# genomematt/xenomapper

Measured on AMD Instinct MI355X. Metric: read-pairs/sec classified, higher is better.
Workload: dtype int32; 1 GPU; configs[1]: 50000000 PE 2x150 pairs/GPU, AS/XS, liberal, HBM-resident; pairs_per_gpu=50000000, step=xm_classify_compact_dev: classify+count, scan, scatter (3 launches)

## Files before the change

### xenomapper_amd/build.py

```python
from __future__ import annotations

import os
import shutil
import subprocess
import sys

PKG = os.path.dirname(os.path.abspath(__file__))
REPO = os.path.dirname(PKG)
CSRC = os.path.join(PKG, "csrc")
HIP_LIB = os.path.join(PKG, "libxenomapper_hip.so")
HOST_LIB = os.path.join(PKG, "libxenomapper_host.so")

HIP_SOURCES = ["xm_kernels.hip", "xm_api.hip", "xm_strip.hip", "xm_inflate.hip", "xm_bamdev.hip"]
HOST_SOURCES = ["xm_sam.cpp", "xm_bam.cpp"]


def _hipcc():
    exe = shutil.which("hipcc") or "/opt/rocm/bin/hipcc"
    if not os.path.exists(exe):
        raise RuntimeError("hipcc not found: the HIP extension cannot be built")
    return exe


def _stale(target, sources):
    if not os.path.exists(target):
        return True
    t = os.path.getmtime(target)
    return any(os.path.getmtime(s) > t for s in sources)


def build_hip(force=False, verbose=False):
    srcs = [os.path.join(CSRC, s) for s in HIP_SOURCES]
    deps = srcs + [os.path.join(CSRC, "xm_kernels.h"), os.path.join(CSRC, "xm_inflate_core.h"),
                   os.path.join(CSRC, "xm_bamrec.h"), os.path.join(CSRC, "xm_fmtg.h"), os.path.join(CSRC, "xm_pinned.h"), os.path.join(CSRC, "xm_gather.h"),
                   os.path.join(REPO, "include", "xenomapper_hip.h"), os.path.join(REPO, "include", "xenomapper_strip.h"),
                   os.path.join(REPO, "include", "xenomapper_bgzf.h")]
    if not force and not _stale(HIP_LIB, deps):
        return HIP_LIB
    flags = ["-O3", "--offload-arch=gfx950", "-std=c++17", "-fPIC", "-Wall", "-Wextra", "-I", os.path.join(REPO, "include")] + \
        os.environ.get("XENOMAPPER_HIPCC_FLAGS", "").split()
    obj_dir = os.path.join(REPO, "build", "obj")
    os.makedirs(obj_dir, exist_ok=True)
    tag = os.path.join(obj_dir, "flags.txt")
    same_flags = os.path.exists(tag) and open(tag).read() == " ".join(flags)
    headers = deps[len(srcs):]
    jobs, objs = [], []
    for src in srcs:
        obj = os.path.join(obj_dir, os.path.basename(src) + ".o")
        objs.append(obj)
        if force or not same_flags or _stale(obj, [src] + headers):
            cmd = [_hipcc()] + flags + ["-c", src, "-o", obj]
            if verbose:
                print(" ".join(cmd), file=sys.stderr)
            jobs.append((cmd, subprocess.Popen(cmd)))
    failed = [cmd for cmd, proc in jobs if proc.wait() != 0]
    if failed:
        raise subprocess.CalledProcessError(1, failed[0])
    with open(tag, "w") as fh:
        fh.write(" ".join(flags))
    cmd = [_hipcc(), "--offload-arch=gfx950", "-shared", "-fPIC"] + objs + ["-o", HIP_LIB]
    if verbose:
        print(" ".join(cmd), file=sys.stderr)
    subprocess.check_call(cmd)
    return HIP_LIB


def build_host(force=False, verbose=False):
    srcs = [os.path.join(CSRC, s) for s in HOST_SOURCES]
    if not all(os.path.exists(s) for s in srcs):
        return None
    deps = srcs + [os.path.join(REPO, "include", "xenomapper_host.h"), os.path.join(CSRC, "xm_pool.h")]
    if not force and not _stale(HOST_LIB, deps):
        return HOST_LIB
    cmd = ["g++", "-O3", "-std=c++17", "-fPIC", "-shared", "-pthread", "-Wall", "-Wextra",
           "-I", os.path.join(REPO, "include")] + srcs + ["-o", HOST_LIB, "-lz", "-ldl"]
    if verbose:
        print(" ".join(cmd), file=sys.stderr)
    subprocess.check_call(cmd)
    return HOST_LIB


def build_host_sanitized(out_path, verbose=False):
    srcs = [os.path.join(CSRC, s) for s in HOST_SOURCES]
    cmd = ["g++", "-O1", "-g", "-std=c++17", "-fPIC", "-shared", "-pthread", "-fsanitize=address,undefined",
           "-fno-omit-frame-pointer", "-I", os.path.join(REPO, "include")] + srcs + ["-o", out_path, "-lz", "-ldl"]
    if verbose:
        print(" ".join(cmd), file=sys.stderr)
    subprocess.check_call(cmd)
    return out_path


def build_all(force=False, verbose=False):
    out = [build_hip(force, verbose)]
    host = build_host(force, verbose)
    if host:
        out.append(host)
    return out


if __name__ == "__main__":
    print("\n".join(build_all(force="--force" in sys.argv, verbose=True)))
```

### xenomapper_amd/csrc/xm_kernels.h

```cpp
#pragma once
#include <hip/hip_runtime.h>
#include <stdint.h>

#include "../../include/xenomapper_hip.h"

#define XM_BLOCK 256
#define XM_GRAN 2048
#define XM_MAX_GRANULES ((uint32_t)((0xFFFFF000ull + XM_GRAN - 1) / XM_GRAN))
#define XM_PART_GRAN 1024u
#define XM_PART_STRIDE 2112u
#define XM_PART_REPLICAS 64u
#define XM_COUNT_REPLICAS 64u
#define XM_CLASSIFY_BLOCK 512
#ifndef XM_CIGAR_BLOCK
#define XM_CIGAR_BLOCK 256
#endif
#define XM_CIGP_BLOCK 512
#ifndef XM_SCATTER_WAVES
#define XM_SCATTER_WAVES 1048576u
#endif
#define XM_CLASSIFY_NT true

namespace xm {

struct GranPlan {
    uint32_t n_gran;
    uint32_t gran_stride;
};

struct CountPlan {
    GranPlan plan = {0, 0};
    uint32_t *gran_counts = nullptr;
    uint32_t *part_tot = nullptr;
    uint8_t *bins4 = nullptr;
    uint64_t *counts_rep = nullptr;
    uint32_t gran0 = 0, gran1 = 0;
};

GranPlan plan_granules(uint64_t n);

struct CigCols {
    const int32_t *nm;
    const int32_t *xs;
    const uint8_t *cnt;
    const uint32_t *tile;
    const uint32_t *ops;
};

struct ListOut {
    uint32_t *p[7];
    uint32_t cap;
};

struct RunsOut {
    uint16_t *runs16;
    uint16_t *gran_counts16;
    uint64_t *counts_rep;
};
void launch_classify_runs_i32(hipStream_t st, int mode, uint64_t n,
                              const int32_t *as1, const int32_t *xs1, const int32_t *as2, const int32_t *xs2,
                              const uint64_t *unit_bits, int32_t m, const RunsOut &ro);
void launch_classify_runs_f64(hipStream_t st, int mode, uint64_t n,
                              const double *as1, const double *xs1, const double *as2, const double *xs2,
                              const uint64_t *unit_bits, double m, const RunsOut &ro);
void launch_runs_finish(hipStream_t st, int mode, uint64_t *counts_rep, uint64_t *counts, uint64_t *n_out);

void launch_classify_i32(hipStream_t st, int mode, uint64_t n,
                         const int32_t *as1, const int32_t *xs1, const int32_t *as2, const int32_t *xs2,
                         const uint64_t *unit_bits, int32_t m, uint8_t *code, const CountPlan *cp);
void launch_classify_f64(hipStream_t st, int mode, uint64_t n,
                         const double *as1, const double *xs1, const double *as2, const double *xs2,
                         const uint64_t *unit_bits, double m, uint8_t *code, const CountPlan *cp);
void launch_classify_cigar(hipStream_t st, int mode, uint64_t n,
                           const int32_t *nm1, const uint32_t *off1, const uint32_t *ops1, const int32_t *xs1,
                           const int32_t *nm2, const uint32_t *off2, const uint32_t *ops2, const int32_t *xs2,
                           const uint64_t *unit_bits, int32_t m, uint8_t *code, uint32_t *range_flag);
void launch_classify_cigp(hipStream_t st, int mode, uint64_t n, const CigCols &s1, const CigCols &s2,
                          const uint64_t *unit_bits, int32_t m, uint8_t *code, uint32_t *range_flag, const CountPlan &cp);
void launch_hist(hipStream_t st, int mode, uint64_t n, const uint8_t *code, const CountPlan &cp);
void launch_scan(hipStream_t st, const CountPlan &cp, uint32_t *gran_off, uint64_t *bin_totals, uint64_t *counts);
void launch_scatter(hipStream_t st, const GranPlan &p, int mode, uint64_t n, const uint8_t *code, bool code_is_bins4,
                    const uint32_t *gran_counts, const uint32_t *gran_off, const uint64_t *bin_totals, uint64_t *bin_offsets,
                    uint32_t *idx_out, uint32_t *part_tot, const ListOut *lists = nullptr, uint32_t gran0 = 0, uint32_t gran1 = 0);
void launch_stream_probe(hipStream_t st, uint64_t n, const int32_t *c0, const int32_t *c1, const int32_t *c2, const int32_t *c3,
                         uint8_t *out);
void launch_mate_correlate(hipStream_t st, uint64_t n, const double *track, uint32_t m, const double *density, double *out);
void launch_cigar(hipStream_t st, uint32_t max_blocks, uint64_t n, const int32_t *nm, const uint32_t *cig_off,
                  const uint32_t *cig_oplen, int32_t *as_out, uint32_t *range_flag);

}
```

### xenomapper_amd/csrc/xm_kernels.hip

```cpp
#include <hip/hip_runtime.h>
#include <stdint.h>
#include <stdlib.h>

#include "xm_kernels.h"

namespace xm {

template <typename T>
__device__ __forceinline__ uint32_t mapping_state(T a1, T x1, T a2, T x2, T m)
{
    const bool low1 = a1 <= m;
    const bool low2 = a2 <= m;
    const bool prim = (a1 > m) && (low2 || a1 > a2);
    const bool sec  = (a2 > m) && (low1 || a2 > a1);
    const bool spec1 = (x1 == T(0)) || (a1 > x1);
    const bool spec2 = (x2 == T(0)) || (a2 > x2);
    uint32_t s = 6u;
    s = sec ? (spec2 ? 1u : 3u) : s;
    s = (a1 == a2) ? 4u : s;
    s = prim ? (spec1 ? 0u : 2u) : s;
    s = (low1 && low2) ? 5u : s;
    return s;
}

template <>
__device__ __forceinline__ uint32_t mapping_state<int32_t>(int32_t a1, int32_t x1, int32_t a2, int32_t x2, int32_t m)
{
    const bool low1 = a1 <= m, low2 = a2 <= m;
    const bool gt = a1 > a2, lt = a2 > a1;
    const bool spec1 = (x1 == 0) || (a1 > x1);
    const bool spec2 = (x2 == 0) || (a2 > x2);
    uint32_t s = spec2 ? 1u : 3u;
    s = (gt || lt) ? s : 4u;
    s = (!low1 && (low2 || gt)) ? (spec1 ? 0u : 2u) : s;
    s = (low1 && low2) ? 5u : s;
    return s;
}

__device__ __forceinline__ uint32_t bin_of_code(int mode, uint32_t c)
{
    const uint32_t f = (c >> 3) & 7u, r = c & 7u;
    const uint32_t lo = f < r ? f : r;
    const uint32_t hi = f < r ? r : f;
    uint32_t b;
    if (mode == XM_MODE_SE) {
        b = r > 6u ? 6u : r;
    } else if (mode == XM_MODE_PE_LIBERAL) {
        b = lo;
    } else {
        b = (hi == 5u) ? 5u
          : ((hi == 4u) || (((f ^ r) & 1u) != 0u)) ? 4u
          : lo;
    }
    if (mode != XM_MODE_SE) b = (hi > 5u) ? 6u : b;
    return (c == XM_NO_UNIT) ? 7u : b;
}

template <typename T> struct Vec4;
typedef int32_t v4i32 __attribute__((ext_vector_type(4)));
typedef int32_t v4i32_a4 __attribute__((ext_vector_type(4), aligned(4)));
typedef double  v4f64 __attribute__((ext_vector_type(4)));
template <> struct Vec4<int32_t> { typedef v4i32 type; };
template <> struct Vec4<double>  { typedef v4f64 type; };

template <typename T> __device__ __forceinline__ T absent_value();
template <> __device__ __forceinline__ int32_t absent_value<int32_t>() { return INT32_MIN; }
template <> __device__ __forceinline__ double  absent_value<double>()  { return -__builtin_huge_val(); }

template <typename T, bool NT, bool FULL = false>
__device__ __forceinline__ void load4(const T *__restrict__ col, uint64_t r0, uint64_t n, T out[4])
{
    typedef typename Vec4<T>::type V;
    if (FULL || r0 + 4 <= n) {
        const V *p = reinterpret_cast<const V *>(col + r0);
        const V v = NT ? __builtin_nontemporal_load(p) : *p;
        out[0] = v.x; out[1] = v.y; out[2] = v.z; out[3] = v.w;
    } else {
#pragma unroll
        for (int j = 0; j < 4; ++j) out[j] = (r0 + j < n) ? col[r0 + j] : absent_value<T>();
    }
}

template <typename T, bool NT>
__device__ __forceinline__ void load4_wg(const T *__restrict__ wg, uint32_t byte_off, T out[4])
{
    typedef typename Vec4<T>::type V;
    const V *p = reinterpret_cast<const V *>(reinterpret_cast<const char *>(wg) + byte_off);
    const V v = NT ? __builtin_nontemporal_load(p) : *p;
    out[0] = v.x; out[1] = v.y; out[2] = v.z; out[3] = v.w;
}

__device__ __forceinline__ uint32_t wave_scan_incl(uint32_t v)
{
    v += (uint32_t)__builtin_amdgcn_update_dpp(0, (int)v, 0x111, 0xf, 0xf, false);
    v += (uint32_t)__builtin_amdgcn_update_dpp(0, (int)v, 0x112, 0xf, 0xf, false);
    v += (uint32_t)__builtin_amdgcn_update_dpp(0, (int)v, 0x114, 0xf, 0xf, false);
    v += (uint32_t)__builtin_amdgcn_update_dpp(0, (int)v, 0x118, 0xf, 0xf, false);
    v += (uint32_t)__builtin_amdgcn_update_dpp(0, (int)v, 0x142, 0xa, 0xf, false);
    v += (uint32_t)__builtin_amdgcn_update_dpp(0, (int)v, 0x143, 0xc, 0xf, false);
    return v;
}

__device__ __forceinline__ uint32_t lane_value(uint32_t v, int lane)
{
    return (uint32_t)__builtin_amdgcn_readlane((int)v, lane);
}

__device__ __forceinline__ void lds_settle()
{
    asm volatile("s_waitcnt lgkmcnt(0)" ::: "memory");
}

#define XM_HREP 8
#define XM_COUNT_LDS_WORDS (64 * XM_HREP + 16)

struct CountSink {
    uint32_t *gran_counts;
    uint32_t *part_tot;
    unsigned long long *counts_rep;
    uint8_t *bins4;
    uint32_t gran_stride;
    int mode;
    uint32_t blk0;
};

__device__ __forceinline__ void count_flush(uint32_t *lds, uint32_t granule, const CountSink &sink)
{
    const uint32_t lane = threadIdx.x & 63u;
    uint32_t *misc = lds + 64 * XM_HREP;
    const uint4 h0 = *reinterpret_cast<const uint4 *>(lds + lane * XM_HREP);
    const uint4 h1 = *reinterpret_cast<const uint4 *>(lds + lane * XM_HREP + 4);
    const uint32_t s = h0.x + h0.y + h0.z + h0.w + h1.x + h1.y + h1.z + h1.w;
    if (s != 0u) {
        atomicAdd(&sink.counts_rep[(granule % XM_COUNT_REPLICAS) * 64u + lane], (unsigned long long)s);
        atomicAdd(&misc[8u + bin_of_code(sink.mode, lane)], s);
    }
    lds_settle();
    if (lane < 8u) {
        const uint32_t v = misc[8u + lane];
        sink.gran_counts[(uint64_t)lane * sink.gran_stride + granule] = v;
        if (v != 0u) atomicAdd(&sink.part_tot[((granule & (XM_PART_REPLICAS - 1u)) * 8u + lane) * XM_PART_STRIDE + granule / XM_PART_GRAN], v);
    }
}

template <int BLOCK>
__device__ __forceinline__ void count_units(const uint32_t c[4], uint32_t *lds, const CountSink &sink)
{
    const uint32_t lane = threadIdx.x & 63u;
    const uint32_t rep = lane & (XM_HREP - 1u);
#pragma unroll
    for (int j = 0; j < 4; ++j) {
        const bool unit = c[j] != XM_NO_UNIT;
        if (__ballot(unit) == 0ull) continue;
        if (unit) atomicAdd(&lds[(c[j] & 63u) * XM_HREP + rep], 1u);
    }
    lds_settle();
    uint32_t arrived = 0;
    if (lane == 0u) arrived = atomicAdd(&lds[64 * XM_HREP], 1u);
    arrived = (uint32_t)__builtin_amdgcn_readfirstlane((int)arrived);
    if (arrived != (uint32_t)(BLOCK / 64 - 1)) return;
    lds_settle();
    count_flush(lds, blockIdx.x + sink.blk0, sink);
}

template <int MODE, bool HAS6>
__device__ __forceinline__ uint32_t unit_bin(uint32_t c)
{
    if (MODE == XM_MODE_SE) return c == XM_NO_UNIT ? 7u : (c & 7u);
    const uint32_t f = (c >> 3) & 7u, r = c & 7u;
    const uint32_t lo = f < r ? f : r, hi = f < r ? r : f;
    uint32_t b = lo;
    if (MODE == XM_MODE_PE_CONSERVATIVE) {
        b = (((f ^ r) & 1u) != 0u || hi == 4u) ? 4u : b;
        b = (hi == 5u) ? 5u : b;
    }
    if (HAS6) b = (hi > 5u) ? 6u : b;
    return c == XM_NO_UNIT ? 7u : b;
}

template <int MODE, bool HAS6>
__device__ __forceinline__ uint32_t unit_bin_of(uint32_t f, uint32_t r, bool unit)
{
    uint32_t b;
    if (MODE == XM_MODE_SE) {
        b = r;
    } else {
        const uint32_t lo = f < r ? f : r, hi = f < r ? r : f;
        b = lo;
        if (MODE == XM_MODE_PE_CONSERVATIVE) {
            b = (((f ^ r) & 1u) != 0u || hi == 4u) ? 4u : b;
            b = (hi == 5u) ? 5u : b;
        }
        if (HAS6) b = (hi > 5u) ? 6u : b;
    }
    return unit ? b : 7u;
}

template <typename T, bool PAIRED, int BLOCK, bool FULL, bool COUNTS, int BINMODE>
__device__ __forceinline__ void classify_finish(const T a1[4], const T x1[4], const T a2[4], const T x2[4], T m,
                                                uint32_t mb, uint32_t halo, uint32_t *last_state,
                                                uint8_t *__restrict__ code, uint64_t r0, uint64_t n,
                                                uint32_t *count_lds, const CountSink &sink)
{
    const uint32_t lane = threadIdx.x & 63u;
    const uint32_t wave = threadIdx.x >> 6;
    uint32_t s[4];
#pragma unroll
    for (int j = 0; j < 4; ++j) s[j] = mapping_state<T>(a1[j], x1[j], a2[j], x2[j], m);

    uint32_t c[4], fwd[4] = {0, 0, 0, 0};
    if (PAIRED) {
        uint32_t prev = (uint32_t)__builtin_amdgcn_update_dpp(0, (int)s[3], 0x138, 0xf, 0xf, false);
        if (lane == 63) last_state[wave] = s[3];
        __syncthreads();
        if (lane == 0) prev = (wave == 0) ? halo : last_state[wave - 1];
        c[0] = (mb & 1u) ? ((prev << 3) | s[0]) : XM_NO_UNIT;
        c[1] = (mb & 2u) ? ((s[0] << 3) | s[1]) : XM_NO_UNIT;
        c[2] = (mb & 4u) ? ((s[1] << 3) | s[2]) : XM_NO_UNIT;
        c[3] = (mb & 8u) ? ((s[2] << 3) | s[3]) : XM_NO_UNIT;
        fwd[0] = prev; fwd[1] = s[0]; fwd[2] = s[1]; fwd[3] = s[2];
    } else {
        if (COUNTS) __syncthreads();
#pragma unroll
        for (int j = 0; j < 4; ++j) c[j] = ((mb >> j) & 1u) ? s[j] : XM_NO_UNIT;
    }

    if (FULL || r0 + 4 <= n) {
        if (code != nullptr) *reinterpret_cast<uint32_t *>(code + r0) = c[0] | (c[1] << 8) | (c[2] << 16) | (c[3] << 24);
    } else {
#pragma unroll
        for (int j = 0; j < 4; ++j)
            if (code != nullptr && r0 + j < n) code[r0 + j] = (uint8_t)c[j];
    }
    if (BINMODE >= 0) {
        uint32_t nib = 0;
#pragma unroll
        for (int j = 0; j < 4; ++j) nib |= unit_bin_of<BINMODE, sizeof(T) == 8>(fwd[j], s[j], ((mb >> j) & 1u) != 0u) << (4 * j);
        reinterpret_cast<uint16_t *>(sink.bins4)[r0 >> 2] = (uint16_t)nib;
    }
    if (COUNTS) count_units<BLOCK>(c, count_lds, sink);
}

template <typename T, bool PAIRED, bool NT, int BLOCK, bool FULL, bool COUNTS, int BINMODE>
__device__ __forceinline__ void classify_body(const T *__restrict__ as1, const T *__restrict__ xs1,
                                              const T *__restrict__ as2, const T *__restrict__ xs2,
                                              const uint8_t *__restrict__ unit_bits8, T m,
                                              uint8_t *__restrict__ code, uint64_t n, uint32_t *last_state,
                                              uint32_t *count_lds, const CountSink &sink)
{
    const uint64_t g = (uint64_t)(blockIdx.x + sink.blk0) * BLOCK + threadIdx.x;
    const uint64_t r0 = g * 4;

    T a1[4], x1[4], a2[4], x2[4];
    load4<T, NT, FULL>(as1, r0, n, a1);
    load4<T, NT, FULL>(xs1, r0, n, x1);
    load4<T, NT, FULL>(as2, r0, n, a2);
    load4<T, NT, FULL>(xs2, r0, n, x2);
    uint32_t mb = 0;
    if (FULL || r0 < n) mb = (uint32_t)(unit_bits8[g >> 1] >> ((g & 1u) * 4u)) & 0xFu;
    if (!FULL && r0 + 4 > n) mb &= (r0 < n) ? ((1u << (uint32_t)(n - r0)) - 1u) : 0u;

    uint32_t halo = 0;
    if (PAIRED && threadIdx.x == 0) {
        if (r0 > 0) {
            const uint64_t h = r0 - 1;
            halo = mapping_state<T>(as1[h], xs1[h], as2[h], xs2[h], m);
        } else {
            mb &= ~1u;
        }
    }
    classify_finish<T, PAIRED, BLOCK, FULL, COUNTS, BINMODE>(a1, x1, a2, x2, m, mb, halo, last_state, code, r0, n, count_lds, sink);
}

template <int BLOCK>
__device__ __forceinline__ void count_lds_clear(uint32_t *count_lds)
{
    for (uint32_t k = threadIdx.x; k < (uint32_t)XM_COUNT_LDS_WORDS; k += BLOCK) count_lds[k] = 0;
}

template <typename T, bool PAIRED, bool NT, int BLOCK, bool COUNTS, int BINMODE>
__global__ void __launch_bounds__(BLOCK)
classify_kernel(const T *__restrict__ as1, const T *__restrict__ xs1,
                const T *__restrict__ as2, const T *__restrict__ xs2,
                const uint8_t *__restrict__ unit_bits8, T m,
                uint8_t *__restrict__ code, uint64_t n, CountSink sink)
{
    __shared__ uint32_t last_state[BLOCK / 64];
    __shared__ __attribute__((aligned(16))) uint32_t count_lds[COUNTS ? XM_COUNT_LDS_WORDS : 4];
    if (COUNTS) count_lds_clear<BLOCK>(count_lds);
    if (((uint64_t)blockIdx.x + sink.blk0 + 1) * (BLOCK * 4) <= n)
        classify_body<T, PAIRED, NT, BLOCK, true, COUNTS, BINMODE>(as1, xs1, as2, xs2, unit_bits8, m, code, n, last_state, count_lds, sink);
    else
        classify_body<T, PAIRED, NT, BLOCK, false, COUNTS, BINMODE>(as1, xs1, as2, xs2, unit_bits8, m, code, n, last_state, count_lds, sink);
}


__device__ __attribute__((noinline)) uint4 load_codes16_tail(const uint8_t *__restrict__ code, uint64_t base, uint64_t n)
{
    uint32_t w[4];
    for (int k = 0; k < 4; ++k) {
        uint32_t acc = 0;
        for (int j = 0; j < 4; ++j) {
            const uint64_t i = base + 4 * k + j;
            const uint32_t c = (i < n) ? (uint32_t)code[i] : XM_NO_UNIT;
            acc |= c << (8 * j);
        }
        w[k] = acc;
    }
    return make_uint4(w[0], w[1], w[2], w[3]);
}

__device__ __forceinline__ void load_codes16(const uint8_t *__restrict__ code, uint64_t base, uint64_t n,
                                             uint32_t w[4])
{
    uint4 v;
    if (base + 16 <= n) v = *reinterpret_cast<const uint4 *>(code + base);
    else v = load_codes16_tail(code, base, n);
    w[0] = v.x; w[1] = v.y; w[2] = v.z; w[3] = v.w;
}

__device__ __attribute__((noinline)) uint32_t load_codes4_tail(const uint8_t *__restrict__ code, uint64_t base, uint64_t n)
{
    uint32_t acc = 0;
    for (int j = 0; j < 4; ++j) {
        const uint64_t i = base + j;
        const uint32_t c = (i < n) ? (uint32_t)code[i] : XM_NO_UNIT;
        acc |= c << (8 * j);
    }
    return acc;
}

__global__ void __launch_bounds__(XM_BLOCK)
hist_kernel(const uint8_t *__restrict__ code, uint64_t n, uint32_t n_gran, CountSink sink)
{
    __shared__ __attribute__((aligned(16))) uint32_t lds_all[XM_BLOCK / 64][XM_COUNT_LDS_WORDS];
    const uint32_t lane = threadIdx.x & 63u, wave = threadIdx.x >> 6;
    uint32_t *lds = lds_all[wave];
    const uint32_t g = blockIdx.x * (XM_BLOCK / 64) + wave;
    if (g >= n_gran) return;
    for (uint32_t k = lane; k < (uint32_t)XM_COUNT_LDS_WORDS; k += 64u) lds[k] = 0;

    constexpr int TILES = XM_GRAN / 1024;
    const uint64_t rec0 = (uint64_t)g * XM_GRAN;
    uint32_t w[TILES][4];
#pragma unroll
    for (int k = 0; k < TILES; ++k) load_codes16(code, rec0 + (uint64_t)k * 1024u + lane * 16u, n, w[k]);
    lds_settle();

    const uint32_t rep = lane & (XM_HREP - 1u);
    uint32_t common = w[0][0] & 0xFFu;
    if (common == XM_NO_UNIT) common = (w[0][0] >> 8) & 0xFFu;
    common = (uint32_t)__builtin_amdgcn_readfirstlane((int)common);
    uint32_t n_common = 0;
#pragma unroll
    for (int k = 0; k < TILES; ++k) {
#pragma unroll
        for (int j = 0; j < 16; ++j) {
            const uint32_t c = (w[k][j >> 2] >> (8 * (j & 3))) & 0xFFu;
            const bool unit = c != XM_NO_UNIT;
            if (__ballot(unit) == 0ull) continue;
            const bool same = unit && c == common;
            n_common += same ? 1u : 0u;
            if (unit && !same) atomicAdd(&lds[(c & 63u) * XM_HREP + rep], 1u);
        }
    }
    if (n_common) atomicAdd(&lds[(common & 63u) * XM_HREP + rep], n_common);
    lds_settle();
    count_flush(lds, g, sink);
}

#define XM_SCAN_THREADS 1024
__device__ __forceinline__ unsigned long long block_sum_1024(unsigned long long v, unsigned long long *wsum)
{
    v += __shfl_xor(v, 1, 64);  v += __shfl_xor(v, 2, 64);  v += __shfl_xor(v, 4, 64);
    v += __shfl_xor(v, 8, 64);  v += __shfl_xor(v, 16, 64); v += __shfl_xor(v, 32, 64);
    if ((threadIdx.x & 63u) == 0u) wsum[threadIdx.x >> 6] = v;
    __syncthreads();
    unsigned long long total = 0;
#pragma unroll
    for (int w = 0; w < XM_SCAN_THREADS / 64; ++w) total += wsum[w];
    return total;
}

__global__ void __launch_bounds__(XM_SCAN_THREADS)
scan_kernel(const uint32_t *__restrict__ gran_counts, uint32_t n_gran, uint32_t gran_stride,
            const uint32_t *__restrict__ part_tot, uint32_t *__restrict__ gran_off,
            unsigned long long *__restrict__ bin_totals,
            unsigned long long *__restrict__ counts_rep, unsigned long long *__restrict__ counts, uint32_t part0, uint32_t n_parts)
{
    __shared__ unsigned long long wsum[XM_SCAN_THREADS / 64];
    __shared__ uint32_t wtot[XM_SCAN_THREADS / 64];
    const uint32_t p = blockIdx.x + part0, b = blockIdx.y;
    const uint32_t t = threadIdx.x, lane = t & 63u, wave = t >> 6;
    if (p + 1u == n_parts && t < 64u) {
        const uint32_t slot = b * 8u + (t >> 3), part = t & 7u;
        unsigned long long acc = 0;
        for (uint32_t r = part; r < XM_COUNT_REPLICAS; r += 8u) {
            acc += counts_rep[r * 64u + slot];
            counts_rep[r * 64u + slot] = 0;
        }
        acc += __shfl_xor(acc, 1, 64);
        acc += __shfl_xor(acc, 2, 64);
        acc += __shfl_xor(acc, 4, 64);
        if (part == 0) counts[slot] = acc;
    }
    const uint32_t g = p * XM_PART_GRAN + t;
    const uint32_t x = (g < n_gran) ? gran_counts[(uint64_t)b * gran_stride + g] : 0u;
    unsigned long long part_sum = 0;
    for (uint32_t e = t; e < p * XM_PART_REPLICAS; e += XM_SCAN_THREADS) {
        const uint32_t r = e / p, q = e - r * p;
        part_sum += part_tot[(r * 8u + b) * XM_PART_STRIDE + q];
    }
    const unsigned long long carry = block_sum_1024(part_sum, wsum);

    const uint32_t incl = wave_scan_incl(x);
    if (lane == 63u) wtot[wave] = incl;
    __syncthreads();
    uint32_t before_wave = 0, part_total = 0;
    for (uint32_t w = 0; w < XM_SCAN_THREADS / 64; ++w) {
        const uint32_t v = wtot[w];
        before_wave += (w < wave) ? v : 0u;
        part_total += v;
    }
    if (g < n_gran) gran_off[(uint64_t)b * gran_stride + g] = (uint32_t)carry + before_wave + incl - x;
    if (p + 1u == n_parts && t == 0u) bin_totals[b] = carry + part_total;
}

#ifndef XM_SCATTER_GUARD
#define XM_SCATTER_GUARD 1
#endif
__device__ __forceinline__ uint32_t mbcnt64(uint64_t mask, uint32_t add)
{
    return __builtin_amdgcn_mbcnt_hi((uint32_t)(mask >> 32), __builtin_amdgcn_mbcnt_lo((uint32_t)mask, add));
}

template <bool WIDE>
__device__ __forceinline__ void store_index(uint32_t *__restrict__ idx_out, uint32_t pos, uint32_t rec)
{
    if (WIDE) idx_out[pos] = rec;
    else *reinterpret_cast<uint32_t *>(reinterpret_cast<char *>(idx_out) + (pos << 2)) = rec;
}

template <int SLOTS, bool WIDE, bool STAGED, bool LISTS = false>
__device__ __forceinline__ void scatter_256(const uint32_t bin[4], const uint32_t rec[4], uint32_t base[7],
                                            uint32_t *__restrict__ idx_out, uint32_t n_units, uint16_t *slab,
                                            const uint64_t *lptr = nullptr)
{
    uint32_t pos[4] = {0, 0, 0, 0};
#pragma unroll
    for (int b = 0; b < 7; ++b) {
        uint64_t m[4], any = 0;
#pragma unroll
        for (int j = 0; j < 4; ++j) {
            m[j] = ((SLOTS >> j) & 1) ? __ballot(bin[j] == (uint32_t)b) : 0ull;
            any |= m[j];
        }
        if (any == 0ull) continue;
        uint32_t t = base[b];
#pragma unroll
        for (int j = 0; j < 4; ++j)
            if ((SLOTS >> j) & 1) t = mbcnt64(m[j], t);
#pragma unroll
        for (int j = 0; j < 4; ++j)
            if ((SLOTS >> j) & 1) pos[j] = (bin[j] == (uint32_t)b) ? t : pos[j];
        uint32_t total = 0;
#pragma unroll
        for (int j = 0; j < 4; ++j)
            if ((SLOTS >> j) & 1) total += (uint32_t)__builtin_popcountll(m[j]);
        base[b] += total;
    }
#pragma unroll
    for (int j = 1; j < 4; ++j)
#pragma unroll
        for (int i = 0; i < j; ++i)
            if (((SLOTS >> j) & 1) && ((SLOTS >> i) & 1)) pos[j] += (bin[i] == bin[j]) ? 1u : 0u;
#pragma unroll
    for (int j = 0; j < 4; ++j)
        if (((SLOTS >> j) & 1) && bin[j] < 7u && (!XM_SCATTER_GUARD || pos[j] < n_units)) {
            if (STAGED) slab[pos[j]] = (uint16_t)rec[j];
            else if (LISTS) {
                uint32_t *list = reinterpret_cast<uint32_t *>(lptr[bin[j]]);
                if (list != nullptr) list[pos[j]] = rec[j];
            }
            else store_index<WIDE>(idx_out, pos[j], rec[j]);
        }
}

#ifndef XM_SCATTER_STAGED
#define XM_SCATTER_STAGED 1
#endif
#define XM_SLAB_U16 (XM_GRAN + 64)
#ifndef XM_STAGE_MIN_UNITS
#define XM_STAGE_MIN_UNITS 1536
#endif

template <bool WIDE>
__device__ __forceinline__ void store_index4(uint32_t *__restrict__ idx_out, uint32_t pos, uint32_t r0, uint32_t r1, uint32_t r2, uint32_t r3)
{
    typedef uint32_t v4u32_a4 __attribute__((ext_vector_type(4), aligned(4)));
    v4u32_a4 v; v.x = r0; v.y = r1; v.z = r2; v.w = r3;
    if (WIDE) *reinterpret_cast<v4u32_a4 *>(idx_out + pos) = v;
    else *reinterpret_cast<v4u32_a4 *>(reinterpret_cast<char *>(idx_out) + (pos << 2)) = v;
}

template <bool WIDE>
__device__ __forceinline__ void scatter_copy_out(const uint16_t *slab, uint32_t L, uint32_t G, uint32_t N, uint32_t rec_g,
                                                 uint32_t *__restrict__ idx_out)
{
    const uint32_t lane = threadIdx.x & 63u;
    if (N < 64u) {
        if (lane < N) store_index<WIDE>(idx_out, G + lane, rec_g + slab[L + lane]);
        return;
    }
    const uint32_t h = (0u - G) & 3u;
    const uint32_t body = (N - h) >> 2;
    const uint32_t t = (N - h) & 3u;
    {
        const bool head = lane < h, tail = lane >= 4u && lane - 4u < t;
        const uint32_t e = head ? lane : h + 4u * body + (lane - 4u);
        if (head || tail) store_index<WIDE>(idx_out, G + e, rec_g + slab[L + e]);
    }
    for (uint32_t c = lane; c < body; c += 64u) {
        const uint32_t e = h + 4u * c;
        const uint2 w = *reinterpret_cast<const uint2 *>(slab + L + e);
        store_index4<WIDE>(idx_out, G + e, rec_g + (w.x & 0xFFFFu), rec_g + (w.x >> 16), rec_g + (w.y & 0xFFFFu), rec_g + (w.y >> 16));
    }
}

template <int NSUB, bool WIDE, bool NIB, bool STAGED, bool LISTS>
__device__ __forceinline__ void scatter_granule(const uint32_t w[NSUB], const uint8_t *lut, uint32_t rec_g, uint32_t base[7],
                                                uint32_t *__restrict__ idx_out, uint32_t n_units, uint16_t *slab, const uint64_t *lptr)
{
    const uint32_t lane = threadIdx.x & 63u;
#pragma unroll
    for (int s = 0; s < NSUB; ++s) {
        const uint32_t rec0 = (STAGED ? 0u : rec_g) + (uint32_t)s * 256u + lane * 4u;
        const uint32_t limit = STAGED ? (uint32_t)XM_SLAB_U16 : n_units;
        uint32_t bin[4];
        bool even_free;
        if (NIB) {
#pragma unroll
            for (int j = 0; j < 4; ++j) bin[j] = (w[s] >> (4 * j)) & 7u;
            even_free = (w[s] & 0x0707u) == 0x0707u;
        } else {
            even_free = (w[s] & 0x00FF00FFu) == 0x00FF00FFu;
        }
        const uint32_t rec[4] = {rec0, rec0 + 1u, rec0 + 2u, rec0 + 3u};
        if (__ballot(!even_free) == 0ull) {
            if (!NIB) { bin[0] = bin[2] = 7u; bin[1] = lut[(w[s] >> 8) & 63u]; bin[3] = lut[(w[s] >> 24) & 63u]; }
            scatter_256<0xA, WIDE, STAGED, LISTS && !STAGED>(bin, rec, base, idx_out, limit, slab, lptr);
            continue;
        }
        if (!NIB) {
#pragma unroll
            for (int j = 0; j < 4; ++j) bin[j] = lut[(w[s] >> (8 * j)) & 63u];
        }
        uint32_t y;
        if (NIB) {
            const uint32_t x = w[s] ^ 0x7777u;
            y = (x | (x >> 1) | (x >> 2)) & 0x1111u;
        } else {
            y = (bin[0] < 7u ? 1u : 0u) | (bin[1] < 7u ? 0x10u : 0u) | (bin[2] < 7u ? 0x100u : 0u) | (bin[3] < 7u ? 0x1000u : 0u);
        }
        if (!STAGED && __ballot(__builtin_popcount(y) > 2) == 0ull) {
            const uint32_t rest = y & (y - 1u);
            const uint32_t c0 = y ? (uint32_t)__builtin_ctz(y) : 0u, c1 = rest ? (uint32_t)__builtin_ctz(rest) : 0u;
            const uint32_t j0 = c0 >> 2, j1 = c1 >> 2;
            uint32_t vb[4] = {7u, 7u, 7u, 7u};
            if (NIB) {
                vb[0] = y ? (w[s] >> c0) & 7u : 7u;
                vb[1] = rest ? (w[s] >> c1) & 7u : 7u;
            } else {
#pragma unroll
                for (int j = 0; j < 4; ++j) {
                    vb[0] = (y && j0 == (uint32_t)j) ? bin[j] : vb[0];
                    vb[1] = (rest && j1 == (uint32_t)j) ? bin[j] : vb[1];
                }
            }
            const uint32_t vrec[4] = {rec0 + j0, rec0 + j1, 0u, 0u};
            scatter_256<0x3, WIDE, STAGED, LISTS>(vb, vrec, base, idx_out, limit, slab, lptr);
        } else {
            scatter_256<0xF, WIDE, STAGED, LISTS && !STAGED>(bin, rec, base, idx_out, limit, slab, lptr);
        }
    }
}

template <int NSUB, bool WIDE, bool NIB, bool STAGE, bool LISTS, bool MULTI>
__global__ void __launch_bounds__(XM_BLOCK)
scatter_kernel(const uint8_t *__restrict__ code, uint64_t n, int mode, uint32_t n_gran, uint32_t gran_stride,
               const uint32_t *__restrict__ gran_counts, const uint32_t *__restrict__ gran_off,
               const unsigned long long *__restrict__ bin_totals,
               unsigned long long *__restrict__ bin_offsets, uint32_t *__restrict__ idx_out, uint32_t *__restrict__ part_tot,
               const ListOut lo, uint32_t gran_per_wave, uint32_t g_first, uint32_t last)
{
    constexpr bool CAN_STAGE = STAGE && XM_SCATTER_STAGED != 0 && NSUB * 256 == XM_GRAN;
    __shared__ uint8_t lut_all[NIB ? 1 : XM_BLOCK / 64][64];
    __shared__ uint64_t lptr_all[LISTS ? XM_BLOCK / 64 : 1][8];
    __shared__ __attribute__((aligned(16))) uint16_t slab_all[CAN_STAGE ? XM_BLOCK / 64 : 1][CAN_STAGE ? XM_SLAB_U16 : 4];
    const uint32_t lane = threadIdx.x & 63u;
    if (last) {
        const uint32_t n_parts = (n_gran + XM_PART_GRAN - 1u) / XM_PART_GRAN, cells = 8u * XM_PART_REPLICAS * n_parts;
        for (uint32_t i = blockIdx.x * XM_BLOCK + threadIdx.x; i < cells; i += gridDim.x * XM_BLOCK)
            part_tot[(i / n_parts) * XM_PART_STRIDE + i % n_parts] = 0u;
    }
    const uint32_t wave = (uint32_t)__builtin_amdgcn_readfirstlane((int)(threadIdx.x >> 6));
    const uint32_t g0 = g_first + (blockIdx.x * (XM_BLOCK / 64) + wave) * (MULTI ? gran_per_wave : 1u);
    if (g0 >= n_gran) return;
    uint8_t *lut = lut_all[NIB ? 0 : wave];
    if (!NIB) lut[lane] = (uint8_t)bin_of_code(mode, lane == 63u ? XM_NO_UNIT : lane);
    uint64_t *lptr = lptr_all[LISTS ? wave : 0];
    if (LISTS && lane < 8u) lptr[lane] = lane < 7u ? (uint64_t)(uintptr_t)lo.p[lane] : 0ull;

    uint32_t lane_base, n_units;
    {
        const uint32_t tot = (lane < 8u) ? (uint32_t)bin_totals[lane] : 0u;
        const uint32_t off = (lane < 7u) ? gran_off[(uint64_t)lane * gran_stride + g0] : 0u;
        const uint32_t bin_start = wave_scan_incl(tot) - tot;
        lane_base = LISTS ? off : bin_start + off;
        n_units = LISTS ? lo.cap : lane_value(bin_start, 7);
        if (g0 == g_first && last && lane < 8u) bin_offsets[lane] = (LISTS && lane < 7u) ? tot : bin_start;
    }
    uint16_t *slab = slab_all[CAN_STAGE ? wave : 0];

    auto load_granule = [&](uint32_t g, uint32_t w[NSUB]) {
        const uint64_t rec_g = (uint64_t)g * (NSUB * 256u);
        if (NIB) {
            const uint16_t *nib = reinterpret_cast<const uint16_t *>(code) + (rec_g >> 2) + lane;
#pragma unroll
            for (int s = 0; s < NSUB; ++s) w[s] = nib[s * 64];
        } else if (rec_g + NSUB * 256u <= n) {
#pragma unroll
            for (int s = 0; s < NSUB; ++s) w[s] = *reinterpret_cast<const uint32_t *>(code + rec_g + s * 256u + lane * 4u);
        } else {
#pragma unroll
            for (int s = 0; s < NSUB; ++s) w[s] = load_codes4_tail(code, rec_g + s * 256u + lane * 4u, n);
        }
    };
    auto slab_layout = [&](uint32_t cnt_g, uint32_t &run_start, uint32_t &run_len) -> bool {
        const uint32_t room = (lane < 7u) ? ((cnt_g + 3u) & ~3u) + 4u : 0u;
        const uint32_t incl_room = wave_scan_incl(room), incl_cnt = wave_scan_incl(cnt_g);
        run_start = incl_room - room + (lane_base & 3u);
        const uint32_t cnt = lane_base < n_units ? (cnt_g < n_units - lane_base ? cnt_g : n_units - lane_base) : 0u;
        run_len = run_start < (uint32_t)XM_SLAB_U16 ? (cnt < XM_SLAB_U16 - run_start ? cnt : XM_SLAB_U16 - run_start) : 0u;
        return lane_value(incl_cnt, 6) >= (uint32_t)XM_STAGE_MIN_UNITS;
    };
    auto copy_runs_out = [&](uint32_t run_start, uint32_t run_len, uint32_t rec_g) {
#pragma unroll
        for (int b = 0; b < 7; ++b) {
            const uint32_t N = lane_value(run_len, b);
            uint32_t *__restrict__ dst = LISTS ? lo.p[b] : idx_out;
            if (N == 0u || dst == nullptr) continue;
            scatter_copy_out<WIDE>(slab, lane_value(run_start, b), lane_value(lane_base, b), N, rec_g, dst);
        }
    };

    if (!MULTI) {
        const uint32_t g = g0;
        uint32_t run_start = 0, run_len = 0;
        bool staged = false;
        if (CAN_STAGE) {
            const uint32_t cnt_g = (lane < 7u) ? gran_counts[(uint64_t)lane * gran_stride + g] : 0u;
            staged = slab_layout(cnt_g, run_start, run_len);
        }
        uint32_t base[7];
#pragma unroll
        for (int b = 0; b < 7; ++b) base[b] = lane_value(staged ? run_start : lane_base, b);
        const uint32_t rec_g = (uint32_t)((uint64_t)g * (NSUB * 256u));
        uint32_t w[NSUB];
        load_granule(g, w);
        if (!NIB || LISTS) lds_settle();
        if (CAN_STAGE && staged) {
            scatter_granule<NSUB, WIDE, NIB, true, LISTS>(w, lut, rec_g, base, idx_out, n_units, slab, lptr);
            lds_settle();
            copy_runs_out(run_start, run_len, rec_g);
        } else {
            scatter_granule<NSUB, WIDE, NIB, false, LISTS>(w, lut, rec_g, base, idx_out, n_units, slab, lptr);
        }
        return;
    }

    const uint32_t g1 = g0 + gran_per_wave < n_gran ? g0 + gran_per_wave : n_gran;
    uint32_t base[7];
#pragma unroll
    for (int b = 0; b < 7; ++b) base[b] = lane_value(lane_base, b);
    uint32_t w[NSUB], wn[NSUB];
    load_granule(g0, w);
    if (!NIB || LISTS) lds_settle();
    for (uint32_t g = g0; g < g1; ++g) {
        if (g + 1u < g1) load_granule(g + 1u, wn);
        const uint32_t rec_g = (uint32_t)((uint64_t)g * (NSUB * 256u));
        bool staged = false;
        uint32_t cnt_g = 0;
        if (CAN_STAGE) {
            cnt_g = (lane < 7u) ? gran_counts[(uint64_t)lane * gran_stride + g] : 0u;
            uint32_t run_start, run_len;
            staged = slab_layout(cnt_g, run_start, run_len);
            if (staged) {
                uint32_t sbase[7];
#pragma unroll
                for (int b = 0; b < 7; ++b) sbase[b] = lane_value(run_start, b);
                scatter_granule<NSUB, WIDE, NIB, true, LISTS>(w, lut, rec_g, sbase, idx_out, n_units, slab, lptr);
                lds_settle();
                copy_runs_out(run_start, run_len, rec_g);
                lds_settle();
            }
        }
        if (!staged) {
            if (CAN_STAGE) {
#pragma unroll
                for (int b = 0; b < 7; ++b) base[b] = lane_value(lane_base, b);
            }
            scatter_granule<NSUB, WIDE, NIB, false, LISTS>(w, lut, rec_g, base, idx_out, n_units, slab, lptr);
        }
        if (CAN_STAGE) lane_base += cnt_g;
#pragma unroll
        for (int s = 0; s < NSUB; ++s) w[s] = wn[s];
    }
}

#define XM_RUNS_WCNT_AT (64 * XM_HREP)
#define XM_RUNS_SLAB_AT (XM_RUNS_WCNT_AT + 64)
#define XM_RUNS_LDS_WORDS (XM_RUNS_SLAB_AT + XM_GRAN / 2)

struct RunsSink {
    uint16_t *runs16;
    uint16_t *gran_counts16;
    unsigned long long *counts_rep;
};

template <int SLOTS, int NB>
__device__ __forceinline__ uint32_t runs_ranks(const uint32_t bin[4], uint32_t pos[4])
{
    const uint32_t lane = threadIdx.x & 63u;
    uint32_t wc = 0;
#pragma unroll
    for (int b = 0; b < NB; ++b) {
        uint64_t m[4], any = 0;
#pragma unroll
        for (int j = 0; j < 4; ++j) {
            m[j] = ((SLOTS >> j) & 1) ? __ballot(bin[j] == (uint32_t)b) : 0ull;
            any |= m[j];
        }
        if (any == 0ull) continue;
        uint32_t t = 0, total = 0;
#pragma unroll
        for (int j = 0; j < 4; ++j)
            if ((SLOTS >> j) & 1) { t = mbcnt64(m[j], t); total += (uint32_t)__builtin_popcountll(m[j]); }
#pragma unroll
        for (int j = 0; j < 4; ++j)
            if ((SLOTS >> j) & 1) pos[j] = (bin[j] == (uint32_t)b) ? t : pos[j];
        wc = (lane == (uint32_t)b) ? total : wc;
    }
#pragma unroll
    for (int j = 1; j < 4; ++j)
#pragma unroll
        for (int i = 0; i < j; ++i)
            if (((SLOTS >> j) & 1) && ((SLOTS >> i) & 1)) pos[j] += (bin[i] == bin[j]) ? 1u : 0u;
    return wc;
}

template <typename T, bool PAIRED, bool NT, int BLOCK, bool FULL, int BINMODE>
__device__ __forceinline__ void classify_runs_body(const T *__restrict__ as1, const T *__restrict__ xs1,
                                                   const T *__restrict__ as2, const T *__restrict__ xs2,
                                                   const uint8_t *__restrict__ unit_bits8, T m, uint64_t n,
                                                   uint32_t *last_state, uint32_t *lds, const RunsSink &rs)
{
    static_assert(BLOCK == 512 && BLOCK * 4 == XM_GRAN, "eight waves, one granule");
    constexpr bool HAS6 = sizeof(T) == 8;
    constexpr int NB = HAS6 ? 7 : 6;
    const uint32_t lane = threadIdx.x & 63u;
    const uint32_t wave = (uint32_t)__builtin_amdgcn_readfirstlane((int)(threadIdx.x >> 6));
    const uint32_t g = blockIdx.x;
    const uint64_t g4 = (uint64_t)blockIdx.x * BLOCK + threadIdx.x;
    const uint64_t r0 = g4 * 4;
    T a1[4], x1[4], a2[4], x2[4];
    load4<T, NT, FULL>(as1, r0, n, a1);
    load4<T, NT, FULL>(xs1, r0, n, x1);
    load4<T, NT, FULL>(as2, r0, n, a2);
    load4<T, NT, FULL>(xs2, r0, n, x2);
    uint32_t mb = 0;
    if (FULL || r0 < n) mb = (uint32_t)(unit_bits8[g4 >> 1] >> ((g4 & 1u) * 4u)) & 0xFu;
    if (!FULL && r0 + 4 > n) mb &= (r0 < n) ? ((1u << (uint32_t)(n - r0)) - 1u) : 0u;
    uint32_t halo = 0;
    if (PAIRED && threadIdx.x == 0) {
        if (r0 > 0) {
            const uint64_t h = r0 - 1;
            halo = mapping_state<T>(as1[h], xs1[h], as2[h], xs2[h], m);
        } else {
            mb &= ~1u;
        }
    }
    uint32_t s[4];
#pragma unroll
    for (int j = 0; j < 4; ++j) s[j] = mapping_state<T>(a1[j], x1[j], a2[j], x2[j], m);
    uint32_t c[4], fwd[4] = {0, 0, 0, 0};
    if (PAIRED) {
        uint32_t prev = (uint32_t)__builtin_amdgcn_update_dpp(0, (int)s[3], 0x138, 0xf, 0xf, false);
        if (lane == 63) last_state[wave] = s[3];
        __syncthreads();
        if (lane == 0) prev = (wave == 0) ? halo : last_state[wave - 1];
        c[0] = (mb & 1u) ? ((prev << 3) | s[0]) : XM_NO_UNIT;
        c[1] = (mb & 2u) ? ((s[0] << 3) | s[1]) : XM_NO_UNIT;
        c[2] = (mb & 4u) ? ((s[1] << 3) | s[2]) : XM_NO_UNIT;
        c[3] = (mb & 8u) ? ((s[2] << 3) | s[3]) : XM_NO_UNIT;
        fwd[0] = prev; fwd[1] = s[0]; fwd[2] = s[1]; fwd[3] = s[2];
    } else {
        __syncthreads();
#pragma unroll
        for (int j = 0; j < 4; ++j) c[j] = ((mb >> j) & 1u) ? s[j] : XM_NO_UNIT;
    }
    uint32_t bin[4];
#pragma unroll
    for (int j = 0; j < 4; ++j) bin[j] = unit_bin_of<BINMODE, HAS6>(fwd[j], s[j], ((mb >> j) & 1u) != 0u);
    {
        const uint32_t rep = lane & (XM_HREP - 1u);
#pragma unroll
        for (int j = 0; j < 4; ++j) {
            const bool unit = c[j] != XM_NO_UNIT;
            if (__ballot(unit) == 0ull) continue;
            if (unit) atomicAdd(&lds[(c[j] & 63u) * XM_HREP + rep], 1u);
        }
    }
    uint32_t pos[4] = {0, 0, 0, 0};
    const bool inter = PAIRED && __ballot((mb & 5u) != 0u) == 0ull;
    const uint32_t wc = inter ? runs_ranks<0xA, NB>(bin, pos) : runs_ranks<0xF, NB>(bin, pos);
    uint32_t *wave_cnt = lds + XM_RUNS_WCNT_AT;
    uint16_t *slab = reinterpret_cast<uint16_t *>(lds + XM_RUNS_SLAB_AT);
    if (lane < 8u) wave_cnt[wave * 8u + lane] = wc;
    __syncthreads();
    uint32_t off, tot;
    {
        const uint32_t v = wave_cnt[lane];
        off = (lane >> 3) < wave ? v : 0u;
        tot = v;
        off += (uint32_t)__shfl_xor((int)off, 8, 64);  tot += (uint32_t)__shfl_xor((int)tot, 8, 64);
        off += (uint32_t)__shfl_xor((int)off, 16, 64); tot += (uint32_t)__shfl_xor((int)tot, 16, 64);
        off += (uint32_t)__shfl_xor((int)off, 32, 64); tot += (uint32_t)__shfl_xor((int)tot, 32, 64);
    }
    const uint32_t t8 = lane < 8u ? tot : 0u;
    const uint32_t incl8 = wave_scan_incl(t8);
    const uint32_t where = incl8 - t8 + off;
    const uint32_t units = lane_value(incl8, 7);
#pragma unroll
    for (int j = 0; j < 4; ++j) {
        uint32_t at = 0;
#pragma unroll
        for (int b = 0; b < NB; ++b) at = (bin[j] == (uint32_t)b) ? lane_value(where, b) : at;
        if (bin[j] < 7u) slab[at + pos[j]] = (uint16_t)(threadIdx.x * 4u + (uint32_t)j);
    }
    __syncthreads();
    if (threadIdx.x < (uint32_t)(XM_GRAN / 8) && threadIdx.x * 8u < units)
        reinterpret_cast<uint4 *>(rs.runs16 + (uint64_t)g * XM_GRAN)[threadIdx.x] = reinterpret_cast<const uint4 *>(slab)[threadIdx.x];
    if (wave == 0u) {
        if (lane < 8u) rs.gran_counts16[(uint64_t)g * 8u + lane] = (uint16_t)tot;
        const uint4 h0 = *reinterpret_cast<const uint4 *>(lds + lane * XM_HREP);
        const uint4 h1 = *reinterpret_cast<const uint4 *>(lds + lane * XM_HREP + 4);
        const uint32_t sum = h0.x + h0.y + h0.z + h0.w + h1.x + h1.y + h1.z + h1.w;
        if (sum != 0u) atomicAdd(&rs.counts_rep[(g % XM_COUNT_REPLICAS) * 64u + lane], (unsigned long long)sum);
    }
}

template <typename T, bool PAIRED, bool NT, int BLOCK, int BINMODE>
__global__ void __launch_bounds__(BLOCK)
classify_runs_kernel(const T *__restrict__ as1, const T *__restrict__ xs1, const T *__restrict__ as2, const T *__restrict__ xs2,
                     const uint8_t *__restrict__ unit_bits8, T m, uint64_t n, RunsSink rs)
{
    __shared__ uint32_t last_state[BLOCK / 64];
    __shared__ __attribute__((aligned(16))) uint32_t lds[XM_RUNS_LDS_WORDS];
    for (uint32_t q = threadIdx.x; q < 64u * XM_HREP; q += BLOCK) lds[q] = 0;
    if (((uint64_t)blockIdx.x + 1) * (BLOCK * 4) <= n)
        classify_runs_body<T, PAIRED, NT, BLOCK, true, BINMODE>(as1, xs1, as2, xs2, unit_bits8, m, n, last_state, lds, rs);
    else
        classify_runs_body<T, PAIRED, NT, BLOCK, false, BINMODE>(as1, xs1, as2, xs2, unit_bits8, m, n, last_state, lds, rs);
}

__global__ void __launch_bounds__(256)
runs_finish_kernel(unsigned long long *__restrict__ counts_rep, unsigned long long *__restrict__ counts,
                   unsigned long long *__restrict__ n_out, int mode)
{
    __shared__ unsigned long long part[4][64];
    __shared__ unsigned long long bins[8];
    const uint32_t slot = threadIdx.x & 63u, q = threadIdx.x >> 6;
    unsigned long long acc = 0;
#pragma unroll
    for (uint32_t r = 0; r < XM_COUNT_REPLICAS / 4u; ++r) {
        acc += counts_rep[(q * (XM_COUNT_REPLICAS / 4u) + r) * 64u + slot];
        counts_rep[(q * (XM_COUNT_REPLICAS / 4u) + r) * 64u + slot] = 0;
    }
    part[q][slot] = acc;
    if (threadIdx.x < 8u) bins[threadIdx.x] = 0;
    __syncthreads();
    if (q == 0u) {
        const unsigned long long v = part[0][slot] + part[1][slot] + part[2][slot] + part[3][slot];
        counts[slot] = v;
        if (v != 0ull) {
            atomicAdd(&bins[bin_of_code(mode, slot)], v);
            atomicAdd(&bins[7], v);
        }
    }
    __syncthreads();
    if (threadIdx.x < 8u) n_out[threadIdx.x] = bins[threadIdx.x];
}

__global__ void __launch_bounds__(XM_BLOCK)
cigar_kernel(uint64_t n, const int32_t *__restrict__ nm, const uint32_t *__restrict__ cig_off,
             const uint32_t *__restrict__ cig_oplen, int32_t *__restrict__ as_out,
             uint32_t *__restrict__ range_flag)
{
    const uint64_t stride = (uint64_t)gridDim.x * XM_BLOCK;
    for (uint64_t i = (uint64_t)blockIdx.x * XM_BLOCK + threadIdx.x; i < n; i += stride) {
        const int32_t nmv = nm[i];
        int32_t out = INT32_MIN;
        if (nmv != INT32_MIN) {
            long long s = -6ll * (long long)nmv;
            const uint32_t k1 = cig_off[i + 1];
            for (uint32_t k = cig_off[i]; k < k1; ++k) {
                const uint32_t v = cig_oplen[k];
                const uint32_t op = v & 15u;
                const long long len = (long long)(v >> 4);
                s -= (op == 1u || op == 2u) ? (5ll + 3ll * len) : 0ll;
                s -= (op == 4u) ? 2ll * len : 0ll;
            }
            if (s <= (long long)INT32_MIN || s > (long long)INT32_MAX) {
                if (range_flag) atomicOr(range_flag, 1u);
                s = s < 0 ? (long long)INT32_MIN + 1 : (long long)INT32_MAX;
            }
            out = (int32_t)s;
        }
        as_out[i] = out;
    }
}

#define XM_CIG_SPEC 3

__device__ __forceinline__ long long cigar_term(uint32_t v)
{
    const uint32_t op = v & 15u;
    const long long len = (long long)(v >> 4);
    long long t = (op == 1u || op == 2u) ? (5ll + 3ll * len) : 0ll;
    t += (op == 4u) ? 2ll * len : 0ll;
    return t;
}

__device__ __forceinline__ uint32_t cigar_term32(uint32_t v)
{
    const uint32_t op = v & 15u, len = v >> 4;
    uint32_t t = (op == 1u || op == 2u) ? (5u + 3u * len) : 0u;
    t += (op == 4u) ? 2u * len : 0u;
    return t;
}

__device__ __forceinline__ uint32_t cigar_term24(uint32_t v)
{
    uint32_t op = v & 15u;
    op = op < 8u ? op : 8u;
    const uint32_t a = __builtin_amdgcn_ubfe(0x00000550u, op * 4u, 4u);
    const uint32_t b = __builtin_amdgcn_ubfe(0x00020330u, op * 4u, 4u);
    return __umul24(b, v >> 4) + a;
}

__device__ __forceinline__ int32_t cigar_clamp(long long s, uint32_t *range_flag)
{
    if (s <= (long long)INT32_MIN || s > (long long)INT32_MAX) {
        if (range_flag) atomicOr(range_flag, 1u);
        s = s < 0 ? (long long)INT32_MIN + 1 : (long long)INT32_MAX;
    }
    return (int32_t)s;
}

__device__ __forceinline__ int32_t cigar_score_one(const int32_t *__restrict__ nm, const uint32_t *__restrict__ off,
                                                   const uint32_t *__restrict__ ops, uint64_t i, uint32_t *range_flag)
{
    const int32_t nmv = nm[i];
    if (nmv == INT32_MIN) return INT32_MIN;
    long long s = -6ll * (long long)nmv;
    const uint32_t k1 = off[i + 1];
    for (uint32_t k = off[i]; k < k1; ++k) s -= cigar_term(ops[k]);
    return cigar_clamp(s, range_flag);
}

struct __attribute__((packed, aligned(4))) Ops3 {
    uint32_t v[XM_CIG_SPEC];
};

template <bool FULL>
__device__ __forceinline__ void cigar_fetch_offsets(const int32_t *__restrict__ nm, const uint32_t *__restrict__ off,
                                                    uint64_t r0, uint64_t n, int32_t nmv[4], uint32_t o[5])
{
    load4<int32_t, true, FULL>(nm, r0, n, nmv);
    if (FULL || r0 + 4 <= n) {
        const v4i32 q = __builtin_nontemporal_load(reinterpret_cast<const v4i32 *>(off + r0));
        o[0] = (uint32_t)q.x; o[1] = (uint32_t)q.y; o[2] = (uint32_t)q.z; o[3] = (uint32_t)q.w;
        o[4] = off[r0 + 4];
    } else {
        uint32_t prev = 0u;
#pragma unroll
        for (int j = 0; j < 5; ++j) {
            const uint32_t v = (r0 + j <= n) ? off[r0 + j] : prev;
            o[j] = v;
            prev = v;
        }
    }
}

__device__ __forceinline__ void cigar_fetch_ops(const uint32_t *__restrict__ ops, uint32_t n_ops, const uint32_t o[5],
                                                uint32_t v[4][XM_CIG_SPEC])
{
    if (__ballot(o[3] + XM_CIG_SPEC > n_ops) == 0ull) {
#pragma unroll
        for (int j = 0; j < 4; ++j) {
            const Ops3 t = *reinterpret_cast<const Ops3 *>(ops + o[j]);
#pragma unroll
            for (int q = 0; q < XM_CIG_SPEC; ++q) v[j][q] = t.v[q];
        }
    } else {
#pragma unroll
        for (int j = 0; j < 4; ++j)
#pragma unroll
            for (int q = 0; q < XM_CIG_SPEC; ++q) v[j][q] = (o[j] + (uint32_t)q < o[j + 1]) ? ops[o[j] + q] : 0u;
    }
}

__device__ __forceinline__ bool cigar_finish_scores(const uint32_t *__restrict__ ops, const int32_t nmv[4], const uint32_t o[5],
                                                    const uint32_t v[4][XM_CIG_SPEC], int32_t as_out[4])
{
    long long s[4];
    bool longer = false;
#pragma unroll
    for (int j = 0; j < 4; ++j) {
        const uint32_t k = o[j + 1] - o[j];
        uint32_t acc = 0;
#pragma unroll
        for (int q = 0; q < XM_CIG_SPEC; ++q) acc += ((uint32_t)q < k) ? cigar_term32(v[j][q]) : 0u;
        s[j] = -6ll * (long long)nmv[j] - (long long)acc;
        longer |= k > (uint32_t)XM_CIG_SPEC;
    }
    if (__ballot(longer) != 0ull) {
#pragma unroll
        for (int j = 0; j < 4; ++j)
            for (uint32_t k = o[j] + XM_CIG_SPEC; k < o[j + 1]; ++k) s[j] -= cigar_term(ops[k]);
    }
    bool bad = false;
#pragma unroll
    for (int j = 0; j < 4; ++j) {
        const bool present = nmv[j] != INT32_MIN;
        const bool out = present && (s[j] <= (long long)INT32_MIN || s[j] > (long long)INT32_MAX);
        bad |= out;
        const long long c = out ? (s[j] < 0 ? (long long)INT32_MIN + 1 : (long long)INT32_MAX) : s[j];
        as_out[j] = present ? (int32_t)c : INT32_MIN;
    }
    return bad;
}

#define XM_CIG_WAVE_OPS 1024
__device__ __forceinline__ bool cigar_scores_by_prefix(const uint32_t *__restrict__ ops, uint32_t n_ops, const int32_t nmv[4],
                                                       const uint32_t o[5], uint32_t *T, int32_t as_out[4], bool &bad)
{
    const uint32_t lane = threadIdx.x & 63u;
    const uint32_t base = __builtin_amdgcn_readfirstlane(o[0]);
    const uint32_t W = lane_value(o[4], 63) - base;
    bool odd = false;
#pragma unroll
    for (int j = 0; j < 4; ++j) odd |= (o[j + 1] - o[j]) > 512u;
    if (W >= (uint32_t)XM_CIG_WAVE_OPS || __ballot(odd) != 0ull) return false;
    uint32_t carry = 0;
    const uint32_t chunks = W / 256u + 1u;
    for (uint32_t c = 0; c < chunks; ++c) {
        const uint32_t s0 = c * 256u + 4u * lane;
        uint32_t v[4];
        if (base + (c + 1u) * 256u <= n_ops) {
            v[0] = v[1] = v[2] = v[3] = 0u;
            if (s0 < W) {
                const v4i32 q = *reinterpret_cast<const v4i32_a4 *>(ops + base + s0);
                v[0] = (uint32_t)q.x; v[1] = (uint32_t)q.y; v[2] = (uint32_t)q.z; v[3] = (uint32_t)q.w;
            }
        } else {
#pragma unroll
            for (int q = 0; q < 4; ++q) v[q] = (base + s0 + (uint32_t)q < n_ops) ? ops[base + s0 + (uint32_t)q] : 0u;
        }
        uint32_t t[4];
#pragma unroll
        for (int q = 0; q < 4; ++q) {
            const bool in = s0 + (uint32_t)q < W;
            odd |= in && (v[q] >> 4) >= (1u << 20);
            t[q] = in ? cigar_term32(v[q]) : 0u;
        }
        const uint32_t p1 = t[0], p2 = p1 + t[1], p3 = p2 + t[2], tot = p3 + t[3];
        const uint32_t incl = wave_scan_incl(tot);
        const uint32_t ex = incl - tot + carry;
        *reinterpret_cast<uint4 *>(T + s0) = make_uint4(ex, ex + p1, ex + p2, ex + p3);
        carry += lane_value(incl, 63);
    }
    if (__ballot(odd) != 0ull) return false;
#pragma unroll
    for (int j = 0; j < 4; ++j) {
        const uint32_t d = T[o[j + 1] - base] - T[o[j] - base];
        const long long sc = -6ll * (long long)nmv[j] - (long long)d;
        const bool present = nmv[j] != INT32_MIN;
        const bool out = present && (sc <= (long long)INT32_MIN || sc > (long long)INT32_MAX);
        bad |= out;
        const long long cl = out ? (sc < 0 ? (long long)INT32_MIN + 1 : (long long)INT32_MAX) : sc;
        as_out[j] = present ? (int32_t)cl : INT32_MIN;
    }
    return true;
}

template <bool PAIRED, int BLOCK, bool FULL>
__device__ __forceinline__ void classify_cigar_body(
    const int32_t *__restrict__ nm1, const uint32_t *__restrict__ off1, const uint32_t *__restrict__ ops1,
    const int32_t *__restrict__ xs1,
    const int32_t *__restrict__ nm2, const uint32_t *__restrict__ off2, const uint32_t *__restrict__ ops2,
    const int32_t *__restrict__ xs2,
    const uint8_t *__restrict__ unit_bits8, int32_t m, uint8_t *__restrict__ code, uint64_t n,
    uint32_t *__restrict__ range_flag, uint32_t *last_state, uint32_t *cig_T)
{
    const uint64_t g = (uint64_t)blockIdx.x * BLOCK + threadIdx.x;
    const uint64_t r0 = g * 4;

    int32_t a1[4], x1[4], a2[4], x2[4];
    load4<int32_t, true, FULL>(xs1, r0, n, x1);
    load4<int32_t, true, FULL>(xs2, r0, n, x2);
    uint32_t mb = 0;
    if (FULL || r0 < n) mb = (uint32_t)(unit_bits8[g >> 1] >> ((g & 1u) * 4u)) & 0xFu;
    if (!FULL && r0 + 4 > n) mb &= (r0 < n) ? ((1u << (uint32_t)(n - r0)) - 1u) : 0u;
    bool bad = false;
    if (FULL || r0 < n) {
        int32_t nmv1[4], nmv2[4];
        uint32_t o1[5], o2[5], v1[4][XM_CIG_SPEC], v2[4][XM_CIG_SPEC];
        const uint32_t n_ops1 = off1[n], n_ops2 = off2[n];
        cigar_fetch_offsets<FULL>(nm1, off1, r0, n, nmv1, o1);
        cigar_fetch_offsets<FULL>(nm2, off2, r0, n, nmv2, o2);
        const bool done1 = FULL && cigar_scores_by_prefix(ops1, n_ops1, nmv1, o1, cig_T, a1, bad);
        const bool done2 = FULL && cigar_scores_by_prefix(ops2, n_ops2, nmv2, o2, cig_T, a2, bad);
        if (!done1) {
            cigar_fetch_ops(ops1, n_ops1, o1, v1);
            bad |= cigar_finish_scores(ops1, nmv1, o1, v1, a1);
        }
        if (!done2) {
            cigar_fetch_ops(ops2, n_ops2, o2, v2);
            bad |= cigar_finish_scores(ops2, nmv2, o2, v2, a2);
        }
    } else {
#pragma unroll
        for (int j = 0; j < 4; ++j) a1[j] = a2[j] = INT32_MIN;
    }
    if (__ballot(bad) != 0ull && (threadIdx.x & 63u) == 0u && range_flag) atomicOr(range_flag, 1u);

    uint32_t halo = 0;
    if (PAIRED && threadIdx.x == 0) {
        if (r0 > 0) {
            const uint64_t h = r0 - 1;
            halo = mapping_state<int32_t>(cigar_score_one(nm1, off1, ops1, h, range_flag), xs1[h],
                                          cigar_score_one(nm2, off2, ops2, h, range_flag), xs2[h], m);
        } else {
            mb &= ~1u;
        }
    }
    const CountSink none = {nullptr, nullptr, nullptr, nullptr, 0u, 0, 0u};
    classify_finish<int32_t, PAIRED, BLOCK, FULL, false, -1>(a1, x1, a2, x2, m, mb, halo, last_state, code, r0, n, nullptr, none);
}

template <bool PAIRED, int BLOCK>
__global__ void __launch_bounds__(BLOCK)
classify_cigar_kernel(const int32_t *__restrict__ nm1, const uint32_t *__restrict__ off1, const uint32_t *__restrict__ ops1,
                      const int32_t *__restrict__ xs1,
                      const int32_t *__restrict__ nm2, const uint32_t *__restrict__ off2, const uint32_t *__restrict__ ops2,
                      const int32_t *__restrict__ xs2,
                      const uint8_t *__restrict__ unit_bits8, int32_t m, uint8_t *__restrict__ code, uint64_t n,
                      uint32_t *__restrict__ range_flag)
{
    __shared__ uint32_t last_state[BLOCK / 64];
    __shared__ __attribute__((aligned(16))) uint32_t cig_table[BLOCK / 64][XM_CIG_WAVE_OPS + 4];
    uint32_t *cig_T = cig_table[threadIdx.x >> 6];
    if (((uint64_t)blockIdx.x + 1) * (BLOCK * 4) <= n)
        classify_cigar_body<PAIRED, BLOCK, true>(nm1, off1, ops1, xs1, nm2, off2, ops2, xs2, unit_bits8, m, code, n,
                                                 range_flag, last_state, cig_T);
    else
        classify_cigar_body<PAIRED, BLOCK, false>(nm1, off1, ops1, xs1, nm2, off2, ops2, xs2, unit_bits8, m, code, n,
                                                  range_flag, last_state, cig_T);
}

#define XM_CIGP_CHUNK 512u

struct TileOps {
    uint32_t tb, te;
    uint32_t v[8];
    bool fast;
    bool brief;
};

__device__ __forceinline__ void cigp_load8(const uint32_t *__restrict__ ops, uint32_t base, uint32_t W, uint32_t s0, uint32_t v[8])
{
    const uint32_t *p = ops + base + ((s0 < W) ? s0 : 0u);
    const v4i32 a = __builtin_nontemporal_load(reinterpret_cast<const v4i32_a4 *>(p));
    const v4i32 b = __builtin_nontemporal_load(reinterpret_cast<const v4i32_a4 *>(p + 4));
    v[0] = (uint32_t)a.x; v[1] = (uint32_t)a.y; v[2] = (uint32_t)a.z; v[3] = (uint32_t)a.w;
    v[4] = (uint32_t)b.x; v[5] = (uint32_t)b.y; v[6] = (uint32_t)b.z; v[7] = (uint32_t)b.w;
}

__device__ __forceinline__ void cigp_load4(const uint32_t *__restrict__ ops, uint32_t base, uint32_t W, uint32_t s0, uint32_t v[8])
{
    const uint32_t *p = ops + base + ((s0 < W) ? s0 : 0u);
    const v4i32 a = __builtin_nontemporal_load(reinterpret_cast<const v4i32_a4 *>(p));
    v[0] = (uint32_t)a.x; v[1] = (uint32_t)a.y; v[2] = (uint32_t)a.z; v[3] = (uint32_t)a.w;
}

__device__ __forceinline__ uint32_t cigp_chunk4(const uint32_t v[8], uint32_t s0, uint32_t *T, uint32_t &any)
{
    uint32_t p[4], run = 0;
#pragma unroll
    for (int q = 0; q < 4; ++q) {
        p[q] = run;
        any |= v[q];
        run += cigar_term24(v[q]);
    }
    const uint32_t tincl = wave_scan_incl(run);
    const uint32_t ex = tincl - run;
    *reinterpret_cast<uint4 *>(T + s0) = make_uint4(ex + p[0], ex + p[1], ex + p[2], ex + p[3]);
    return lane_value(tincl, 63);
}

__device__ __forceinline__ uint32_t cigp_chunk(const uint32_t v[8], uint32_t s0, uint32_t carry, uint32_t *T, uint32_t &any)
{
    uint32_t p[8], run = 0;
#pragma unroll
    for (int q = 0; q < 8; ++q) {
        p[q] = run;
        any |= v[q];
        run += cigar_term24(v[q]);
    }
    const uint32_t tincl = wave_scan_incl(run);
    const uint32_t ex = tincl - run + carry;
    *reinterpret_cast<uint4 *>(T + s0) = make_uint4(ex + p[0], ex + p[1], ex + p[2], ex + p[3]);
    *reinterpret_cast<uint4 *>(T + s0 + 4u) = make_uint4(ex + p[4], ex + p[5], ex + p[6], ex + p[7]);
    return carry + lane_value(tincl, 63);
}

__device__ __forceinline__ bool cigp_fast(const uint32_t *__restrict__ ops, const TileOps &o, uint32_t cw,
                                          const int32_t nmv[4], uint32_t *T, int32_t as_out[4], bool &bad)
{
    const uint32_t lane = threadIdx.x & 63u;
    const uint32_t W = o.te - o.tb;
    const uint32_t c0 = cw & 255u, c1 = (cw >> 8) & 255u, c2 = (cw >> 16) & 255u, c3 = cw >> 24;
    const uint32_t lsum = c0 + c1 + c2 + c3;
    const uint32_t incl = wave_scan_incl(lsum);
    const bool esc = c0 == 255u || c1 == 255u || c2 == 255u || c3 == 255u;
    if (lane_value(incl, 63) != W || __ballot(esc) != 0ull) return false;
    uint32_t any = 0;
    uint32_t carry = o.brief ? cigp_chunk4(o.v, 4u * lane, T, any) : cigp_chunk(o.v, 8u * lane, 0u, T, any);
    if (W >= XM_CIGP_CHUNK) {
        uint32_t v[8];
        cigp_load8(ops, o.tb, W, XM_CIGP_CHUNK + 8u * lane, v);
        carry = cigp_chunk(v, XM_CIGP_CHUNK + 8u * lane, carry, T, any);
    }
    const bool odd = any >= (1u << 24);
    if (__ballot(odd) != 0ull) return false;
    const uint32_t b0 = incl - lsum, b1 = b0 + c0, b2 = b1 + c1, b3 = b2 + c2, b4 = b3 + c3;
    const uint32_t t0 = T[b0], t1 = T[b1], t2 = T[b2], t3 = T[b3], t4 = T[b4];
    const uint32_t d[4] = {t1 - t0, t2 - t1, t3 - t2, t4 - t3};
    bool big = false;
#pragma unroll
    for (int j = 0; j < 4; ++j) {
        const bool present = nmv[j] != INT32_MIN;
        const int32_t nme = present ? nmv[j] : 0;
        big |= (uint32_t)(nme + (1 << 23)) >= (1u << 24) || d[j] >= (1u << 30);
        as_out[j] = present ? __mul24(nme, -6) - (int32_t)d[j] : INT32_MIN;
    }
    (void)bad;
    return __ballot(big) == 0ull;
}

__device__ __forceinline__ int32_t cigp_score_range(const uint32_t *__restrict__ ops, uint32_t n_ops, int32_t nmv,
                                                    uint32_t b, uint32_t e, uint32_t *range_flag)
{
    if (nmv == INT32_MIN) return INT32_MIN;
    long long s = -6ll * (long long)nmv;
    if (e > n_ops) e = n_ops;
    for (uint32_t k = b; k < e; ++k) s -= cigar_term(ops[k]);
    return cigar_clamp(s, range_flag);
}

__device__ __forceinline__ uint32_t cigp_trailer(const uint32_t *__restrict__ ops, uint32_t n_ops, uint32_t end)
{
    return (end > 0u && end <= n_ops) ? (ops[end - 1u] >> 4) : 0u;
}

__device__ __forceinline__ v4i32 cigp_slow(const uint32_t *__restrict__ ops, uint32_t n_ops, uint32_t tb, uint32_t te,
                                                     uint32_t cw, v4i32 nmv, uint32_t *range_flag)
{
    const uint32_t lane = threadIdx.x & 63u;
    if (te > n_ops) te = n_ops;
    if (tb > te) tb = te;
    const uint32_t c0 = cw & 255u, c1 = (cw >> 8) & 255u, c2 = (cw >> 16) & 255u, c3 = cw >> 24;
    uint32_t b0, b1, b2, b3, e0, e1, e2, e3;
    if (__ballot(c0 == 255u || c1 == 255u || c2 == 255u || c3 == 255u) == 0ull) {
        const uint32_t lsum = c0 + c1 + c2 + c3;
        b0 = tb + wave_scan_incl(lsum) - lsum;
        e0 = b1 = b0 + c0; e1 = b2 = b1 + c1; e2 = b3 = b2 + c2; e3 = b3 + c3;
    } else {
        b0 = b1 = b2 = b3 = e0 = e1 = e2 = e3 = tb;
        uint32_t end = te;
        for (int L = 63; L >= 0; --L) {
            const uint32_t w = lane_value(cw, L);
#pragma unroll
            for (int j = 3; j >= 0; --j) {
                uint32_t k = (w >> (8 * j)) & 255u, e = end;
                if (k == 255u) { k = cigp_trailer(ops, n_ops, end); e = end > tb ? end - 1u : tb; }
                const uint32_t b = (e - tb >= k) ? e - k : tb;
                if (lane == (uint32_t)L) {
                    if (j == 0) { b0 = b; e0 = e; } else if (j == 1) { b1 = b; e1 = e; }
                    else if (j == 2) { b2 = b; e2 = e; } else { b3 = b; e3 = e; }
                }
                end = b;
            }
        }
    }
    v4i32 r;
    r.x = cigp_score_range(ops, n_ops, nmv.x, b0, e0, range_flag);
    r.y = cigp_score_range(ops, n_ops, nmv.y, b1, e1, range_flag);
    r.z = cigp_score_range(ops, n_ops, nmv.z, b2, e2, range_flag);
    r.w = cigp_score_range(ops, n_ops, nmv.w, b3, e3, range_flag);
    return r;
}

__device__ __attribute__((noinline)) int32_t cigp_score_before(const int32_t *__restrict__ nm, const uint8_t *__restrict__ cnt,
                                                               const uint32_t *__restrict__ ops, uint32_t n_ops, uint64_t h,
                                                               uint32_t end, uint32_t *range_flag)
{
    if (end > n_ops) end = n_ops;
    uint32_t k = cnt[h], e = end;
    if (k == 255u) { k = cigp_trailer(ops, n_ops, end); e = end > 0u ? end - 1u : 0u; }
    return cigp_score_range(ops, n_ops, nm[h], e >= k ? e - k : 0u, e, range_flag);
}

template <bool FULL>
__device__ __forceinline__ uint32_t cigp_counts4(const uint8_t *__restrict__ cnt, uint64_t r0, uint64_t n)
{
    if (FULL || r0 + 4 <= n) return __builtin_nontemporal_load(reinterpret_cast<const uint32_t *>(cnt + r0));
    uint32_t w = 0;
#pragma unroll
    for (int j = 0; j < 4; ++j)
        if (r0 + j < n) w |= (uint32_t)cnt[r0 + j] << (8 * j);
    return w;
}

template <bool PAIRED, int BLOCK, bool FULL, bool COUNTS, int BINMODE>
__device__ __forceinline__ void classify_cigp_body(const CigCols s1, const CigCols s2, const uint8_t *__restrict__ unit_bits8,
                                                   int32_t m, uint8_t *__restrict__ code, uint64_t n, uint32_t n_tiles,
                                                   uint32_t *__restrict__ range_flag, uint32_t *last_state, uint32_t *cig_T,
                                                   uint32_t *count_lds, const CountSink &sink)
{
    const uint32_t wave = (uint32_t)__builtin_amdgcn_readfirstlane((int)(threadIdx.x >> 6));
    const uint32_t t = blockIdx.x * (BLOCK / 64) + wave;
    const uint64_t g = (uint64_t)blockIdx.x * BLOCK + threadIdx.x;
    const uint64_t r0 = g * 4;
    const bool have_tile = FULL || t < n_tiles;
    const uint32_t lane = threadIdx.x & 63u;

    int32_t a1[4], x1[4], a2[4], x2[4], nmv1[4], nmv2[4];
    uint32_t cw1, cw2, mb = 0;
    const uint64_t wg0 = (uint64_t)blockIdx.x * (BLOCK * 4);
    const uint32_t t16 = threadIdx.x * 16u, t4 = threadIdx.x * 4u;
    if (FULL) {
        load4_wg<int32_t, true>(s1.nm + wg0, t16, nmv1);
        load4_wg<int32_t, true>(s2.nm + wg0, t16, nmv2);
        cw1 = __builtin_nontemporal_load(reinterpret_cast<const uint32_t *>(s1.cnt + wg0 + t4));
        cw2 = __builtin_nontemporal_load(reinterpret_cast<const uint32_t *>(s2.cnt + wg0 + t4));
    } else {
        load4<int32_t, true, false>(s1.nm, r0, n, nmv1);
        load4<int32_t, true, false>(s2.nm, r0, n, nmv2);
        cw1 = cigp_counts4<false>(s1.cnt, r0, n);
        cw2 = cigp_counts4<false>(s2.cnt, r0, n);
    }
    TileOps o1, o2;
    o1.tb = o1.te = o2.tb = o2.te = 0u;
    const uint32_t n_ops1 = s1.tile[n_tiles], n_ops2 = s2.tile[n_tiles];
    if (have_tile) { o1.tb = s1.tile[t]; o1.te = s1.tile[t + 1u]; o2.tb = s2.tile[t]; o2.te = s2.tile[t + 1u]; }
    o1.fast = FULL && o1.te >= o1.tb && o1.te - o1.tb < (uint32_t)XM_CIG_WAVE_OPS && (uint64_t)o1.te + 8u <= n_ops1;
    o2.fast = FULL && o2.te >= o2.tb && o2.te - o2.tb < (uint32_t)XM_CIG_WAVE_OPS && (uint64_t)o2.te + 8u <= n_ops2;
#ifndef XM_CIGP_BRIEF
#define XM_CIGP_BRIEF 1
#endif
    o1.brief = XM_CIGP_BRIEF && o1.fast && o1.te - o1.tb < 256u;
    o2.brief = XM_CIGP_BRIEF && o2.fast && o2.te - o2.tb < 256u;
    if (o1.brief) cigp_load4(s1.ops, o1.tb, o1.te - o1.tb, 4u * lane, o1.v);
    else if (o1.fast) cigp_load8(s1.ops, o1.tb, o1.te - o1.tb, 8u * lane, o1.v);
    if (o2.brief) cigp_load4(s2.ops, o2.tb, o2.te - o2.tb, 4u * lane, o2.v);
    else if (o2.fast) cigp_load8(s2.ops, o2.tb, o2.te - o2.tb, 8u * lane, o2.v);

    bool bad = false;
    if (!(o1.fast && cigp_fast(s1.ops, o1, cw1, nmv1, cig_T, a1, bad))) {
        v4i32 q; q.x = nmv1[0]; q.y = nmv1[1]; q.z = nmv1[2]; q.w = nmv1[3];
        q = cigp_slow(s1.ops, n_ops1, o1.tb, o1.te, cw1, q, range_flag);
        a1[0] = q.x; a1[1] = q.y; a1[2] = q.z; a1[3] = q.w;
    }
    if (FULL) {
        load4_wg<int32_t, true>(s1.xs + wg0, t16, x1);
        load4_wg<int32_t, true>(s2.xs + wg0, t16, x2);
        mb = (uint32_t)((unit_bits8 + (wg0 >> 3))[threadIdx.x >> 1] >> ((threadIdx.x & 1u) * 4u)) & 0xFu;
    } else {
        load4<int32_t, true, false>(s1.xs, r0, n, x1);
        load4<int32_t, true, false>(s2.xs, r0, n, x2);
        if (r0 < n) mb = (uint32_t)(unit_bits8[g >> 1] >> ((g & 1u) * 4u)) & 0xFu;
        if (r0 + 4 > n) mb &= (r0 < n) ? ((1u << (uint32_t)(n - r0)) - 1u) : 0u;
    }
    if (!(o2.fast && cigp_fast(s2.ops, o2, cw2, nmv2, cig_T, a2, bad))) {
        v4i32 q; q.x = nmv2[0]; q.y = nmv2[1]; q.z = nmv2[2]; q.w = nmv2[3];
        q = cigp_slow(s2.ops, n_ops2, o2.tb, o2.te, cw2, q, range_flag);
        a2[0] = q.x; a2[1] = q.y; a2[2] = q.z; a2[3] = q.w;
    }
    if (__ballot(bad) != 0ull && (threadIdx.x & 63u) == 0u && range_flag) atomicOr(range_flag, 1u);

    uint32_t halo = 0;
    if (PAIRED && threadIdx.x == 0) {
        if (r0 == 0) {
            mb &= ~1u;
        } else if (mb & 1u) {
            const uint64_t h = r0 - 1;
            halo = mapping_state<int32_t>(cigp_score_before(s1.nm, s1.cnt, s1.ops, n_ops1, h, o1.tb, range_flag), s1.xs[h],
                                          cigp_score_before(s2.nm, s2.cnt, s2.ops, n_ops2, h, o2.tb, range_flag), s2.xs[h], m);
        }
    }
    classify_finish<int32_t, PAIRED, BLOCK, FULL, COUNTS, BINMODE>(a1, x1, a2, x2, m, mb, halo, last_state, code, r0, n,
                                                                   count_lds, sink);
}

template <bool PAIRED, int BLOCK, bool COUNTS, int BINMODE>
__global__ void __launch_bounds__(BLOCK)
classify_cigp_kernel(const CigCols s1, const CigCols s2, const uint8_t *__restrict__ unit_bits8, int32_t m,
                     uint8_t *__restrict__ code, uint64_t n, uint32_t n_tiles, uint32_t *__restrict__ range_flag, CountSink sink)
{
    static_assert(!COUNTS || BLOCK * 4 == XM_GRAN, "the counting workgroup is one granule");
    __shared__ uint32_t last_state[BLOCK / 64];
    __shared__ __attribute__((aligned(16))) uint32_t cig_table[BLOCK / 64][XM_CIG_WAVE_OPS + 8];
    __shared__ __attribute__((aligned(16))) uint32_t count_lds[COUNTS ? XM_COUNT_LDS_WORDS : 4];
    uint32_t *cig_T = cig_table[threadIdx.x >> 6];
    if (COUNTS) count_lds_clear<BLOCK>(count_lds);
    if (((uint64_t)blockIdx.x + 1) * (BLOCK * 4) <= n)
        classify_cigp_body<PAIRED, BLOCK, true, COUNTS, BINMODE>(s1, s2, unit_bits8, m, code, n, n_tiles, range_flag, last_state,
                                                                 cig_T, count_lds, sink);
    else
        classify_cigp_body<PAIRED, BLOCK, false, COUNTS, BINMODE>(s1, s2, unit_bits8, m, code, n, n_tiles, range_flag, last_state,
                                                                  cig_T, count_lds, sink);
}

#define XM_CORR_T 256
#define XM_CORR_M 2048
__global__ void __launch_bounds__(XM_CORR_T)
mate_correlate_kernel(const double *__restrict__ track, uint64_t n, const double *__restrict__ density, uint32_t m,
                      double *__restrict__ out)
{
#pragma clang fp contract(off)
    __shared__ double tile[XM_CORR_T + XM_CORR_M];
    const uint32_t t = threadIdx.x;
    const uint64_t i0 = (uint64_t)blockIdx.x * XM_CORR_T, i = i0 + t;
    const uint64_t left = (i < n) ? n - i : 0;
    double acc = 0.0;
    for (uint32_t j0 = 0; j0 < m; j0 += XM_CORR_M) {
        const uint32_t mm = (m - j0 < XM_CORR_M) ? m - j0 : XM_CORR_M;
        __syncthreads();
        for (uint32_t k = t; k < XM_CORR_T + mm; k += XM_CORR_T) {
            const uint64_t p = i0 + j0 + k;
            tile[k] = (p < n) ? track[p] : 0.0;
        }
        __syncthreads();
        const uint32_t lim = (left > j0) ? (uint32_t)((left - j0 < mm) ? left - j0 : mm) : 0u;
        if (__ballot(lim != mm) == 0ull) {
            for (uint32_t j = 0; j < mm; ++j) {
                const double prod = tile[t + j] * density[j0 + j];
                acc = acc + prod;
            }
        } else {
            for (uint32_t j = 0; j < mm; ++j) {
                const double prod = tile[t + j] * density[j0 + j];
                const double s = acc + prod;
                acc = (j < lim) ? s : acc;
            }
        }
    }
    if (i < n) out[i] = (track[i] == 1.0) ? 1.0 : acc;
}

__global__ void __launch_bounds__(XM_CLASSIFY_BLOCK)
stream_probe_kernel(const v4i32 *__restrict__ c0, const v4i32 *__restrict__ c1, const v4i32 *__restrict__ c2,
                    const v4i32 *__restrict__ c3, uint16_t *__restrict__ out, uint64_t n_groups)
{
    const uint64_t g = (uint64_t)blockIdx.x * XM_CLASSIFY_BLOCK + threadIdx.x;
    if (g >= n_groups) return;
    const v4i32 a = __builtin_nontemporal_load(c0 + g), b = __builtin_nontemporal_load(c1 + g);
    const v4i32 c = __builtin_nontemporal_load(c2 + g), d = __builtin_nontemporal_load(c3 + g);
    const v4i32 x = a ^ b ^ c ^ d;
    out[g] = (uint16_t)(x.x ^ x.y ^ x.z ^ x.w);
}

void launch_stream_probe(hipStream_t st, uint64_t n, const int32_t *c0, const int32_t *c1, const int32_t *c2, const int32_t *c3,
                         uint8_t *out)
{
    const uint64_t n_groups = n / 4;
    const uint32_t grid = (uint32_t)((n_groups + XM_CLASSIFY_BLOCK - 1) / XM_CLASSIFY_BLOCK);
    if (grid == 0) return;
    stream_probe_kernel<<<grid, XM_CLASSIFY_BLOCK, 0, st>>>(reinterpret_cast<const v4i32 *>(c0), reinterpret_cast<const v4i32 *>(c1),
                                                            reinterpret_cast<const v4i32 *>(c2), reinterpret_cast<const v4i32 *>(c3),
                                                            reinterpret_cast<uint16_t *>(out), n_groups);
}

static_assert(XM_CLASSIFY_BLOCK * 4 == XM_GRAN, "the counting classify workgroup is one granule");

GranPlan plan_granules(uint64_t n)
{
    GranPlan p;
    uint64_t g = (n + XM_GRAN - 1) / XM_GRAN;
    if (g == 0) g = 1;
    p.n_gran = (uint32_t)g;
    p.gran_stride = (p.n_gran + 63u) & ~63u;
    return p;
}

static CountSink make_sink(const CountPlan *cp, int mode)
{
    CountSink s;
    s.gran_counts = cp ? cp->gran_counts : nullptr;
    s.part_tot = cp ? cp->part_tot : nullptr;
    s.counts_rep = cp ? reinterpret_cast<unsigned long long *>(cp->counts_rep) : nullptr;
    s.bins4 = cp ? cp->bins4 : nullptr;
    s.gran_stride = cp ? cp->plan.gran_stride : 0u;
    s.mode = mode;
    s.blk0 = cp ? cp->gran0 : 0u;
    return s;
}

template <typename T>
static void launch_classify_t(hipStream_t st, int mode, uint64_t n,
                              const T *as1, const T *xs1, const T *as2, const T *xs2,
                              const uint64_t *unit_bits, T m, uint8_t *code, const CountPlan *cp)
{
    const uint64_t per_block = (uint64_t)XM_CLASSIFY_BLOCK * 4;
    static_assert(XM_CLASSIFY_BLOCK * 4 == XM_GRAN, "a counting workgroup is a granule: CountPlan's chunk is in both");
    const uint32_t all = (uint32_t)((n + per_block - 1) / per_block);
    const uint32_t grid = (cp && cp->gran1) ? cp->gran1 - cp->gran0 : all;
    const uint8_t *bits8 = reinterpret_cast<const uint8_t *>(unit_bits);
    const CountSink sink = make_sink(cp, mode);
    const bool paired = mode != XM_MODE_SE;
#define XM_LAUNCH_CLS(P, C, B) classify_kernel<T, P, XM_CLASSIFY_NT, XM_CLASSIFY_BLOCK, C, B><<<grid, XM_CLASSIFY_BLOCK, 0, st>>>(as1, xs1, as2, xs2, bits8, m, code, n, sink)
    if (cp && cp->bins4) {
        if (mode == XM_MODE_SE) XM_LAUNCH_CLS(false, true, XM_MODE_SE);
        else if (mode == XM_MODE_PE_LIBERAL) XM_LAUNCH_CLS(true, true, XM_MODE_PE_LIBERAL);
        else XM_LAUNCH_CLS(true, true, XM_MODE_PE_CONSERVATIVE);
    }
    else if (cp) { if (paired) XM_LAUNCH_CLS(true, true, -1); else XM_LAUNCH_CLS(false, true, -1); }
    else         { if (paired) XM_LAUNCH_CLS(true, false, -1); else XM_LAUNCH_CLS(false, false, -1); }
#undef XM_LAUNCH_CLS
}

void launch_classify_i32(hipStream_t st, int mode, uint64_t n,
                         const int32_t *as1, const int32_t *xs1, const int32_t *as2, const int32_t *xs2,
                         const uint64_t *unit_bits, int32_t m, uint8_t *code, const CountPlan *cp)
{
    launch_classify_t<int32_t>(st, mode, n, as1, xs1, as2, xs2, unit_bits, m, code, cp);
}

void launch_classify_f64(hipStream_t st, int mode, uint64_t n,
                         const double *as1, const double *xs1, const double *as2, const double *xs2,
                         const uint64_t *unit_bits, double m, uint8_t *code, const CountPlan *cp)
{
    launch_classify_t<double>(st, mode, n, as1, xs1, as2, xs2, unit_bits, m, code, cp);
}

template <typename T>
static void launch_classify_runs_t(hipStream_t st, int mode, uint64_t n,
                                   const T *as1, const T *xs1, const T *as2, const T *xs2,
                                   const uint64_t *unit_bits, T m, const RunsOut &ro)
{
    const uint64_t per_block = (uint64_t)XM_CLASSIFY_BLOCK * 4;
    const uint32_t grid = (uint32_t)((n + per_block - 1) / per_block);
    const uint8_t *bits8 = reinterpret_cast<const uint8_t *>(unit_bits);
    RunsSink rs;
    rs.runs16 = ro.runs16;
    rs.gran_counts16 = ro.gran_counts16;
    rs.counts_rep = reinterpret_cast<unsigned long long *>(ro.counts_rep);
#define XM_LAUNCH_RUNS(P, B) classify_runs_kernel<T, P, XM_CLASSIFY_NT, XM_CLASSIFY_BLOCK, B><<<grid, XM_CLASSIFY_BLOCK, 0, st>>>(as1, xs1, as2, xs2, bits8, m, n, rs)
    if (mode == XM_MODE_SE) XM_LAUNCH_RUNS(false, XM_MODE_SE);
    else if (mode == XM_MODE_PE_LIBERAL) XM_LAUNCH_RUNS(true, XM_MODE_PE_LIBERAL);
    else XM_LAUNCH_RUNS(true, XM_MODE_PE_CONSERVATIVE);
#undef XM_LAUNCH_RUNS
}

void launch_classify_runs_i32(hipStream_t st, int mode, uint64_t n,
                              const int32_t *as1, const int32_t *xs1, const int32_t *as2, const int32_t *xs2,
                              const uint64_t *unit_bits, int32_t m, const RunsOut &ro)
{
    launch_classify_runs_t<int32_t>(st, mode, n, as1, xs1, as2, xs2, unit_bits, m, ro);
}

void launch_classify_runs_f64(hipStream_t st, int mode, uint64_t n,
                              const double *as1, const double *xs1, const double *as2, const double *xs2,
                              const uint64_t *unit_bits, double m, const RunsOut &ro)
{
    launch_classify_runs_t<double>(st, mode, n, as1, xs1, as2, xs2, unit_bits, m, ro);
}

void launch_runs_finish(hipStream_t st, int mode, uint64_t *counts_rep, uint64_t *counts, uint64_t *n_out)
{
    runs_finish_kernel<<<1, 256, 0, st>>>(reinterpret_cast<unsigned long long *>(counts_rep),
                                          reinterpret_cast<unsigned long long *>(counts),
                                          reinterpret_cast<unsigned long long *>(n_out), mode);
}

void launch_classify_cigar(hipStream_t st, int mode, uint64_t n,
                           const int32_t *nm1, const uint32_t *off1, const uint32_t *ops1, const int32_t *xs1,
                           const int32_t *nm2, const uint32_t *off2, const uint32_t *ops2, const int32_t *xs2,
                           const uint64_t *unit_bits, int32_t m, uint8_t *code, uint32_t *range_flag)
{
    const uint64_t per_block = (uint64_t)XM_CIGAR_BLOCK * 4;
    const uint32_t grid = (uint32_t)((n + per_block - 1) / per_block);
    const uint8_t *bits8 = reinterpret_cast<const uint8_t *>(unit_bits);
    if (mode == XM_MODE_SE)
        classify_cigar_kernel<false, XM_CIGAR_BLOCK><<<grid, XM_CIGAR_BLOCK, 0, st>>>(
            nm1, off1, ops1, xs1, nm2, off2, ops2, xs2, bits8, m, code, n, range_flag);
    else
        classify_cigar_kernel<true, XM_CIGAR_BLOCK><<<grid, XM_CIGAR_BLOCK, 0, st>>>(
            nm1, off1, ops1, xs1, nm2, off2, ops2, xs2, bits8, m, code, n, range_flag);
}

void launch_classify_cigp(hipStream_t st, int mode, uint64_t n, const CigCols &s1, const CigCols &s2,
                          const uint64_t *unit_bits, int32_t m, uint8_t *code, uint32_t *range_flag, const CountPlan &cp)
{
    const uint64_t per_block = (uint64_t)XM_CIGP_BLOCK * 4;
    const uint32_t grid = (uint32_t)((n + per_block - 1) / per_block);
    const uint32_t n_tiles = (uint32_t)((n + 255) / 256);
    const uint8_t *bits8 = reinterpret_cast<const uint8_t *>(unit_bits);
    const CountSink sink = make_sink(&cp, mode);
#define XM_LAUNCH_CIGP(P, B) classify_cigp_kernel<P, XM_CIGP_BLOCK, true, B><<<grid, XM_CIGP_BLOCK, 0, st>>>(s1, s2, bits8, m, code, n, n_tiles, range_flag, sink)
    if (cp.bins4) {
        if (mode == XM_MODE_SE) XM_LAUNCH_CIGP(false, XM_MODE_SE);
        else if (mode == XM_MODE_PE_LIBERAL) XM_LAUNCH_CIGP(true, XM_MODE_PE_LIBERAL);
        else XM_LAUNCH_CIGP(true, XM_MODE_PE_CONSERVATIVE);
    } else {
        if (mode == XM_MODE_SE) XM_LAUNCH_CIGP(false, -1); else XM_LAUNCH_CIGP(true, -1);
    }
#undef XM_LAUNCH_CIGP
}

void launch_hist(hipStream_t st, int mode, uint64_t n, const uint8_t *code, const CountPlan &cp)
{
    const uint32_t grid = (cp.plan.n_gran + (XM_BLOCK / 64) - 1) / (XM_BLOCK / 64);
    hist_kernel<<<grid, XM_BLOCK, 0, st>>>(code, n, cp.plan.n_gran, make_sink(&cp, mode));
}

void launch_scan(hipStream_t st, const CountPlan &cp, uint32_t *gran_off, uint64_t *bin_totals, uint64_t *counts)
{
    const uint32_t n_parts = (cp.plan.n_gran + XM_PART_GRAN - 1) / XM_PART_GRAN;
    unsigned long long *bt = reinterpret_cast<unsigned long long *>(bin_totals);
    unsigned long long *rep = reinterpret_cast<unsigned long long *>(cp.counts_rep);
    unsigned long long *cnt = reinterpret_cast<unsigned long long *>(counts);
    const uint32_t part0 = cp.gran1 ? cp.gran0 / XM_PART_GRAN : 0u;
    const uint32_t part1 = cp.gran1 ? (cp.gran1 + XM_PART_GRAN - 1) / XM_PART_GRAN : n_parts;
    scan_kernel<<<dim3(part1 - part0, 8), XM_SCAN_THREADS, 0, st>>>(cp.gran_counts, cp.gran1 ? cp.gran1 : cp.plan.n_gran, cp.plan.gran_stride,
                                                                   cp.part_tot, gran_off, bt, rep, cnt, part0, n_parts);
}

static uint32_t scatter_waves()
{
    const char *e = getenv("XM_SCATTER_WAVES");
    const long v = e && *e ? strtol(e, nullptr, 10) : 0;
    return v >= 1 && v < (long)XM_SCATTER_WAVES ? (uint32_t)v : (uint32_t)XM_SCATTER_WAVES;
}

void launch_scatter(hipStream_t st, const GranPlan &p, int mode, uint64_t n, const uint8_t *code, bool code_is_bins4,
                    const uint32_t *gran_counts, const uint32_t *gran_off, const uint64_t *bin_totals, uint64_t *bin_offsets,
                    uint32_t *idx_out, uint32_t *part_tot, const ListOut *lists, uint32_t gran0, uint32_t gran1)
{
    const unsigned long long *bt = reinterpret_cast<const unsigned long long *>(bin_totals);
    unsigned long long *bo = reinterpret_cast<unsigned long long *>(bin_offsets);
    const uint32_t g_first = gran1 ? gran0 : 0u, g_end = gran1 ? gran1 : p.n_gran, span = g_end - g_first;
    const uint32_t last = g_end == p.n_gran ? 1u : 0u;
    const uint32_t max_waves = scatter_waves();
    const uint32_t gran_per_wave = (span + max_waves - 1u) / max_waves;
    const bool multi = gran_per_wave > 1u;
    const uint32_t n_waves = multi ? (span + gran_per_wave - 1u) / gran_per_wave : span;
    const uint32_t grid = (n_waves + (XM_BLOCK / 64) - 1) / (XM_BLOCK / 64);
    const bool wide = n > (1ull << 30);
    const bool stage = mode == XM_MODE_SE;
    const ListOut lo = lists ? *lists : ListOut{{nullptr, nullptr, nullptr, nullptr, nullptr, nullptr, nullptr}, 0u};
#define XM_LAUNCH_SCT(W, NIB, STG, L, M) scatter_kernel<XM_GRAN / 256, W, NIB, STG, L, M><<<grid, XM_BLOCK, 0, st>>>(code, n, mode, g_end, p.gran_stride, gran_counts, gran_off, bt, bo, idx_out, part_tot, lo, gran_per_wave, g_first, last)
#define XM_LAUNCH_SCT0(W, NIB, STG, L) do { if (multi) XM_LAUNCH_SCT(W, NIB, STG, L, true); else XM_LAUNCH_SCT(W, NIB, STG, L, false); } while (0)
#define XM_LAUNCH_SCT1(W, NIB, STG) do { if (lists) XM_LAUNCH_SCT0(W, NIB, STG, true); else XM_LAUNCH_SCT0(W, NIB, STG, false); } while (0)
#define XM_LAUNCH_SCT2(W, NIB) do { if (stage) XM_LAUNCH_SCT1(W, NIB, true); else XM_LAUNCH_SCT1(W, NIB, false); } while (0)
    if (code_is_bins4) { if (wide) XM_LAUNCH_SCT2(true, true); else XM_LAUNCH_SCT2(false, true); }
    else               { if (wide) XM_LAUNCH_SCT2(true, false); else XM_LAUNCH_SCT2(false, false); }
#undef XM_LAUNCH_SCT2
#undef XM_LAUNCH_SCT1
#undef XM_LAUNCH_SCT0
#undef XM_LAUNCH_SCT
}

void launch_mate_correlate(hipStream_t st, uint64_t n, const double *track, uint32_t m, const double *density, double *out)
{
    const uint32_t grid = (uint32_t)((n + XM_CORR_T - 1) / XM_CORR_T);
    mate_correlate_kernel<<<grid, XM_CORR_T, 0, st>>>(track, n, density, m, out);
}

void launch_cigar(hipStream_t st, uint32_t max_blocks, uint64_t n, const int32_t *nm, const uint32_t *cig_off,
                  const uint32_t *cig_oplen, int32_t *as_out, uint32_t *range_flag)
{
    uint64_t blocks = (n + XM_BLOCK - 1) / XM_BLOCK;
    if (blocks > max_blocks) blocks = max_blocks;
    if (blocks == 0) blocks = 1;
    cigar_kernel<<<(uint32_t)blocks, XM_BLOCK, 0, st>>>(n, nm, cig_off, cig_oplen, as_out, range_flag);
}

}
```

Baseline: 143.8 billion read-pairs/s.

## Rank scatter bins with packed wave scans and make granule counts granule-major

Replaces the per-bin ballot/mbcnt loop in the scatter with a packed multi-bin prefix scan. Each bin gets a 9-bit field in a 64-bit word, plus a separate word for bin 6, and the wave scans that to rank all four slots at once; a bpermute then fetches the per-bin base. Gran_counts and gran_off move from a bin-major strided layout to granule-major, 8 entries per granule, so each scatter wave reads one contiguous line. Also skips the halo classify load when the first unit bit is unset, folds the scan block reduction into a single barrier, and sets waves_per_eu hints. The packed fields assume per-tile counts fit in 9 bits, and the rewrite carries correctness risk.

```diff
diff --git a/xenomapper_amd/build.py b/xenomapper_amd/build.py
--- a/xenomapper_amd/build.py
+++ b/xenomapper_amd/build.py
@@ -31,7 +31,7 @@
 
 def build_hip(force=False, verbose=False):
     srcs = [os.path.join(CSRC, s) for s in HIP_SOURCES]
-    deps = srcs + [os.path.join(CSRC, "xm_kernels.h"), os.path.join(CSRC, "xm_inflate_core.h"),
+    deps = srcs + [os.path.join(CSRC, "xm_kernels.h"), os.path.join(CSRC, "xm_ranks.h"), os.path.join(CSRC, "xm_inflate_core.h"),
                    os.path.join(CSRC, "xm_bamrec.h"), os.path.join(CSRC, "xm_fmtg.h"), os.path.join(CSRC, "xm_pinned.h"), os.path.join(CSRC, "xm_gather.h"),
                    os.path.join(REPO, "include", "xenomapper_hip.h"), os.path.join(REPO, "include", "xenomapper_strip.h"),
                    os.path.join(REPO, "include", "xenomapper_bgzf.h")]
diff --git a/xenomapper_amd/csrc/xm_kernels.h b/xenomapper_amd/csrc/xm_kernels.h
--- a/xenomapper_amd/csrc/xm_kernels.h
+++ b/xenomapper_amd/csrc/xm_kernels.h
@@ -25,11 +25,10 @@
 
 struct GranPlan {
     uint32_t n_gran;
-    uint32_t gran_stride;
 };
 
 struct CountPlan {
-    GranPlan plan = {0, 0};
+    GranPlan plan = {0};
     uint32_t *gran_counts = nullptr;
     uint32_t *part_tot = nullptr;
     uint8_t *bins4 = nullptr;
diff --git a/xenomapper_amd/csrc/xm_kernels.hip b/xenomapper_amd/csrc/xm_kernels.hip
--- a/xenomapper_amd/csrc/xm_kernels.hip
+++ b/xenomapper_amd/csrc/xm_kernels.hip
@@ -3,6 +3,7 @@
 #include <stdlib.h>
 
 #include "xm_kernels.h"
+#include "xm_ranks.h"
 
 namespace xm {
 
@@ -119,7 +120,6 @@
     uint32_t *part_tot;
     unsigned long long *counts_rep;
     uint8_t *bins4;
-    uint32_t gran_stride;
     int mode;
     uint32_t blk0;
 };
@@ -138,7 +138,7 @@
     lds_settle();
     if (lane < 8u) {
         const uint32_t v = misc[8u + lane];
-        sink.gran_counts[(uint64_t)lane * sink.gran_stride + granule] = v;
+        sink.gran_counts[(uint64_t)granule * 8u + lane] = v;
         if (v != 0u) atomicAdd(&sink.part_tot[((granule & (XM_PART_REPLICAS - 1u)) * 8u + lane) * XM_PART_STRIDE + granule / XM_PART_GRAN], v);
     }
 }
@@ -241,6 +241,9 @@
     if (COUNTS) count_units<BLOCK>(c, count_lds, sink);
 }
 
+#ifndef XM_HALO_WHEN_USED
+#define XM_HALO_WHEN_USED 1
+#endif
 template <typename T, bool PAIRED, bool NT, int BLOCK, bool FULL, bool COUNTS, int BINMODE>
 __device__ __forceinline__ void classify_body(const T *__restrict__ as1, const T *__restrict__ xs1,
                                               const T *__restrict__ as2, const T *__restrict__ xs2,
@@ -250,6 +253,9 @@
 {
     const uint64_t g = (uint64_t)(blockIdx.x + sink.blk0) * BLOCK + threadIdx.x;
     const uint64_t r0 = g * 4;
+
+    static_assert(BLOCK % 8 == 0, "whole mask words per workgroup");
+    const uint32_t first_bits = PAIRED ? reinterpret_cast<const uint32_t *>(unit_bits8)[(uint64_t)(blockIdx.x + sink.blk0) * (BLOCK / 8)] : 0u;
 
     T a1[4], x1[4], a2[4], x2[4];
     load4<T, NT, FULL>(as1, r0, n, a1);
@@ -261,13 +267,10 @@
     if (!FULL && r0 + 4 > n) mb &= (r0 < n) ? ((1u << (uint32_t)(n - r0)) - 1u) : 0u;
 
     uint32_t halo = 0;
-    if (PAIRED && threadIdx.x == 0) {
-        if (r0 > 0) {
-            const uint64_t h = r0 - 1;
-            halo = mapping_state<T>(as1[h], xs1[h], as2[h], xs2[h], m);
-        } else {
-            mb &= ~1u;
-        }
+    if (PAIRED && r0 == 0) mb &= ~1u;
+    if (PAIRED && threadIdx.x == 0 && r0 > 0 && (!XM_HALO_WHEN_USED || (first_bits & 1u))) {
+        const uint64_t h = r0 - 1;
+        halo = mapping_state<T>(as1[h], xs1[h], as2[h], xs2[h], m);
     }
     classify_finish<T, PAIRED, BLOCK, FULL, COUNTS, BINMODE>(a1, x1, a2, x2, m, mb, halo, last_state, code, r0, n, count_lds, sink);
 }
@@ -370,20 +373,9 @@
 }
 
 #define XM_SCAN_THREADS 1024
-__device__ __forceinline__ unsigned long long block_sum_1024(unsigned long long v, unsigned long long *wsum)
-{
-    v += __shfl_xor(v, 1, 64);  v += __shfl_xor(v, 2, 64);  v += __shfl_xor(v, 4, 64);
-    v += __shfl_xor(v, 8, 64);  v += __shfl_xor(v, 16, 64); v += __shfl_xor(v, 32, 64);
-    if ((threadIdx.x & 63u) == 0u) wsum[threadIdx.x >> 6] = v;
-    __syncthreads();
-    unsigned long long total = 0;
-#pragma unroll
-    for (int w = 0; w < XM_SCAN_THREADS / 64; ++w) total += wsum[w];
-    return total;
-}
-
+static_assert(XM_SCAN_THREADS == XM_PART_GRAN, "a thread per granule of the part");
 __global__ void __launch_bounds__(XM_SCAN_THREADS)
-scan_kernel(const uint32_t *__restrict__ gran_counts, uint32_t n_gran, uint32_t gran_stride,
+scan_kernel(const uint32_t *__restrict__ gran_counts, uint32_t n_gran,
             const uint32_t *__restrict__ part_tot, uint32_t *__restrict__ gran_off,
             unsigned long long *__restrict__ bin_totals,
             unsigned long long *__restrict__ counts_rep, unsigned long long *__restrict__ counts, uint32_t part0, uint32_t n_parts)
@@ -405,24 +397,27 @@
         if (part == 0) counts[slot] = acc;
     }
     const uint32_t g = p * XM_PART_GRAN + t;
-    const uint32_t x = (g < n_gran) ? gran_counts[(uint64_t)b * gran_stride + g] : 0u;
+    const uint32_t x = (g < n_gran) ? gran_counts[(uint64_t)g * 8u + b] : 0u;
     unsigned long long part_sum = 0;
     for (uint32_t e = t; e < p * XM_PART_REPLICAS; e += XM_SCAN_THREADS) {
         const uint32_t r = e / p, q = e - r * p;
         part_sum += part_tot[(r * 8u + b) * XM_PART_STRIDE + q];
     }
-    const unsigned long long carry = block_sum_1024(part_sum, wsum);
-
+    part_sum += __shfl_xor(part_sum, 1, 64);  part_sum += __shfl_xor(part_sum, 2, 64);  part_sum += __shfl_xor(part_sum, 4, 64);
+    part_sum += __shfl_xor(part_sum, 8, 64);  part_sum += __shfl_xor(part_sum, 16, 64); part_sum += __shfl_xor(part_sum, 32, 64);
+    if (lane == 0u) wsum[wave] = part_sum;
     const uint32_t incl = wave_scan_incl(x);
     if (lane == 63u) wtot[wave] = incl;
     __syncthreads();
+    unsigned long long carry = 0;
     uint32_t before_wave = 0, part_total = 0;
     for (uint32_t w = 0; w < XM_SCAN_THREADS / 64; ++w) {
         const uint32_t v = wtot[w];
+        carry += wsum[w];
         before_wave += (w < wave) ? v : 0u;
         part_total += v;
     }
-    if (g < n_gran) gran_off[(uint64_t)b * gran_stride + g] = (uint32_t)carry + before_wave + incl - x;
+    if (g < n_gran) gran_off[(uint64_t)g * 8u + b] = (uint32_t)carry + before_wave + incl - x;
     if (p + 1u == n_parts && t == 0u) bin_totals[b] = carry + part_total;
 }
 
@@ -439,51 +434,6 @@
 {
     if (WIDE) idx_out[pos] = rec;
     else *reinterpret_cast<uint32_t *>(reinterpret_cast<char *>(idx_out) + (pos << 2)) = rec;
-}
-
-template <int SLOTS, bool WIDE, bool STAGED, bool LISTS = false>
-__device__ __forceinline__ void scatter_256(const uint32_t bin[4], const uint32_t rec[4], uint32_t base[7],
-                                            uint32_t *__restrict__ idx_out, uint32_t n_units, uint16_t *slab,
-                                            const uint64_t *lptr = nullptr)
-{
-    uint32_t pos[4] = {0, 0, 0, 0};
-#pragma unroll
-    for (int b = 0; b < 7; ++b) {
-        uint64_t m[4], any = 0;
-#pragma unroll
-        for (int j = 0; j < 4; ++j) {
-            m[j] = ((SLOTS >> j) & 1) ? __ballot(bin[j] == (uint32_t)b) : 0ull;
-            any |= m[j];
-        }
-        if (any == 0ull) continue;
-        uint32_t t = base[b];
-#pragma unroll
-        for (int j = 0; j < 4; ++j)
-            if ((SLOTS >> j) & 1) t = mbcnt64(m[j], t);
-#pragma unroll
-        for (int j = 0; j < 4; ++j)
-            if ((SLOTS >> j) & 1) pos[j] = (bin[j] == (uint32_t)b) ? t : pos[j];
-        uint32_t total = 0;
-#pragma unroll
-        for (int j = 0; j < 4; ++j)
-            if ((SLOTS >> j) & 1) total += (uint32_t)__builtin_popcountll(m[j]);
-        base[b] += total;
-    }
-#pragma unroll
-    for (int j = 1; j < 4; ++j)
-#pragma unroll
-        for (int i = 0; i < j; ++i)
-            if (((SLOTS >> j) & 1) && ((SLOTS >> i) & 1)) pos[j] += (bin[i] == bin[j]) ? 1u : 0u;
-#pragma unroll
-    for (int j = 0; j < 4; ++j)
-        if (((SLOTS >> j) & 1) && bin[j] < 7u && (!XM_SCATTER_GUARD || pos[j] < n_units)) {
-            if (STAGED) slab[pos[j]] = (uint16_t)rec[j];
-            else if (LISTS) {
-                uint32_t *list = reinterpret_cast<uint32_t *>(lptr[bin[j]]);
-                if (list != nullptr) list[pos[j]] = rec[j];
-            }
-            else store_index<WIDE>(idx_out, pos[j], rec[j]);
-        }
 }
 
 #ifndef XM_SCATTER_STAGED
@@ -494,6 +444,43 @@
 #define XM_STAGE_MIN_UNITS 1536
 #endif
 
+struct IndexSink {
+    uint32_t *idx_out;
+    uint32_t n_units;
+    uint16_t *slab;
+    const uint64_t *lptr;
+};
+
+template <int SLOTS, bool HAS6, bool WIDE, bool STAGED, bool LISTS>
+__device__ __forceinline__ void scatter_tile(const uint32_t bin[4], uint32_t rec0, uint32_t &place, const IndexSink &to)
+{
+    const uint32_t lane = threadIdx.x & 63u;
+    uint32_t rank[4];
+    const PackedUnits incl = tile_ranks<SLOTS, HAS6>(bin, rank, [](uint32_t v) { return wave_scan_incl(v); });
+    const uint32_t from = place;
+    PackedUnits tot;
+    tot.lo = lane_value(incl.lo, 63); tot.hi = lane_value(incl.hi, 63); tot.b6 = HAS6 ? lane_value(incl.b6, 63) : 0u;
+    place = from + place_advance<HAS6>(tot, lane);
+    uint32_t pos[4];
+#pragma unroll
+    for (int j = 0; j < 4; ++j)
+        if ((SLOTS >> j) & 1) pos[j] = (uint32_t)__builtin_amdgcn_ds_bpermute((int)(bin[j] << 2), (int)from) + rank[j];
+#pragma unroll
+    for (int j = 0; j < 4; ++j) {
+        if (!((SLOTS >> j) & 1)) continue;
+        const uint32_t rec = rec0 + (uint32_t)j;
+        const bool ok = bin[j] < 7u && (!XM_SCATTER_GUARD || pos[j] < to.n_units);
+        if (STAGED) {
+            to.slab[ok ? pos[j] : (uint32_t)XM_SLAB_U16] = (uint16_t)rec;
+        } else if (LISTS) {
+            uint32_t *list = reinterpret_cast<uint32_t *>(to.lptr[bin[j]]);
+            if (ok && list != nullptr) list[pos[j]] = rec;
+        } else {
+            if (ok) store_index<WIDE>(to.idx_out, pos[j], rec);
+        }
+    }
+}
+
 template <bool WIDE>
 __device__ __forceinline__ void store_index4(uint32_t *__restrict__ idx_out, uint32_t pos, uint32_t r0, uint32_t r1, uint32_t r2, uint32_t r3)
 {
@@ -527,67 +514,48 @@
     }
 }
 
+template <int SLOTS, bool HAS6, int NSUB, bool WIDE, bool NIB, bool STAGED, bool LISTS>
+__device__ __forceinline__ void scatter_tiles(const uint32_t w[NSUB], const uint8_t *lut, uint32_t rec_g, uint32_t &place,
+                                              const IndexSink &to)
+{
+    const uint32_t lane = threadIdx.x & 63u;
+#pragma unroll
+    for (int s = 0; s < NSUB; ++s) {
+        uint32_t bin[4] = {7u, 7u, 7u, 7u};
+#pragma unroll
+        for (int j = 0; j < 4; ++j)
+            if ((SLOTS >> j) & 1) bin[j] = NIB ? (w[s] >> (4 * j)) & 7u : lut[(w[s] >> (8 * j)) & 63u];
+        scatter_tile<SLOTS, HAS6, WIDE, STAGED, LISTS>(bin, (STAGED ? 0u : rec_g) + (uint32_t)s * 256u + lane * 4u, place, to);
+    }
+}
+
 template <int NSUB, bool WIDE, bool NIB, bool STAGED, bool LISTS>
-__device__ __forceinline__ void scatter_granule(const uint32_t w[NSUB], const uint8_t *lut, uint32_t rec_g, uint32_t base[7],
-                                                uint32_t *__restrict__ idx_out, uint32_t n_units, uint16_t *slab, const uint64_t *lptr)
-{
-    const uint32_t lane = threadIdx.x & 63u;
+__device__ __forceinline__ void scatter_granule(const uint32_t w[NSUB], const uint8_t *lut, uint32_t rec_g, uint32_t &place,
+                                                const IndexSink &to)
+{
+    bool even_free = true, six = false;
 #pragma unroll
     for (int s = 0; s < NSUB; ++s) {
-        const uint32_t rec0 = (STAGED ? 0u : rec_g) + (uint32_t)s * 256u + lane * 4u;
-        const uint32_t limit = STAGED ? (uint32_t)XM_SLAB_U16 : n_units;
-        uint32_t bin[4];
-        bool even_free;
         if (NIB) {
-#pragma unroll
-            for (int j = 0; j < 4; ++j) bin[j] = (w[s] >> (4 * j)) & 7u;
-            even_free = (w[s] & 0x0707u) == 0x0707u;
+            even_free = even_free && (w[s] & 0x0707u) == 0x0707u;
+            const uint32_t x = w[s] ^ 0x6666u;
+            six = six || (((x | (x >> 1) | (x >> 2)) & 0x1111u) != 0x1111u);
         } else {
-            even_free = (w[s] & 0x00FF00FFu) == 0x00FF00FFu;
-        }
-        const uint32_t rec[4] = {rec0, rec0 + 1u, rec0 + 2u, rec0 + 3u};
-        if (__ballot(!even_free) == 0ull) {
-            if (!NIB) { bin[0] = bin[2] = 7u; bin[1] = lut[(w[s] >> 8) & 63u]; bin[3] = lut[(w[s] >> 24) & 63u]; }
-            scatter_256<0xA, WIDE, STAGED, LISTS && !STAGED>(bin, rec, base, idx_out, limit, slab, lptr);
-            continue;
-        }
-        if (!NIB) {
-#pragma unroll
-            for (int j = 0; j < 4; ++j) bin[j] = lut[(w[s] >> (8 * j)) & 63u];
-        }
-        uint32_t y;
-        if (NIB) {
-            const uint32_t x = w[s] ^ 0x7777u;
-            y = (x | (x >> 1) | (x >> 2)) & 0x1111u;
-        } else {
-            y = (bin[0] < 7u ? 1u : 0u) | (bin[1] < 7u ? 0x10u : 0u) | (bin[2] < 7u ? 0x100u : 0u) | (bin[3] < 7u ? 0x1000u : 0u);
-        }
-        if (!STAGED && __ballot(__builtin_popcount(y) > 2) == 0ull) {
-            const uint32_t rest = y & (y - 1u);
-            const uint32_t c0 = y ? (uint32_t)__builtin_ctz(y) : 0u, c1 = rest ? (uint32_t)__builtin_ctz(rest) : 0u;
-            const uint32_t j0 = c0 >> 2, j1 = c1 >> 2;
-            uint32_t vb[4] = {7u, 7u, 7u, 7u};
-            if (NIB) {
-                vb[0] = y ? (w[s] >> c0) & 7u : 7u;
-                vb[1] = rest ? (w[s] >> c1) & 7u : 7u;
-            } else {
-#pragma unroll
-                for (int j = 0; j < 4; ++j) {
-                    vb[0] = (y && j0 == (uint32_t)j) ? bin[j] : vb[0];
-                    vb[1] = (rest && j1 == (uint32_t)j) ? bin[j] : vb[1];
-                }
-            }
-            const uint32_t vrec[4] = {rec0 + j0, rec0 + j1, 0u, 0u};
-            scatter_256<0x3, WIDE, STAGED, LISTS>(vb, vrec, base, idx_out, limit, slab, lptr);
-        } else {
-            scatter_256<0xF, WIDE, STAGED, LISTS && !STAGED>(bin, rec, base, idx_out, limit, slab, lptr);
-        }
-    }
+            even_free = even_free && (w[s] & 0x00FF00FFu) == 0x00FF00FFu;
+            const uint32_t t = w[s] & (w[s] >> 1), u = t & (t >> 1);
+            six = six || ((((t >> 1) | (t >> 4)) & ~(u & (u >> 3)) & 0x01010101u) != 0u);
+        }
+    }
+    const bool inter = __ballot(!even_free) == 0ull, has6 = __ballot(six) != 0ull;
+#define XM_TILES(S, H) scatter_tiles<S, H, NSUB, WIDE, NIB, STAGED, LISTS>(w, lut, rec_g, place, to)
+    if (inter) { if (has6) XM_TILES(0xA, true); else XM_TILES(0xA, false); }
+    else       { if (has6) XM_TILES(0xF, true); else XM_TILES(0xF, false); }
+#undef XM_TILES
 }
 
 template <int NSUB, bool WIDE, bool NIB, bool STAGE, bool LISTS, bool MULTI>
-__global__ void __launch_bounds__(XM_BLOCK)
-scatter_kernel(const uint8_t *__restrict__ code, uint64_t n, int mode, uint32_t n_gran, uint32_t gran_stride,
+__global__ void __launch_bounds__(XM_BLOCK) __attribute__((amdgpu_waves_per_eu(MULTI ? 1 : 8)))
+scatter_kernel(const uint8_t *__restrict__ code, uint64_t n, int mode, uint32_t n_gran,
                const uint32_t *__restrict__ gran_counts, const uint32_t *__restrict__ gran_off,
                const unsigned long long *__restrict__ bin_totals,
                unsigned long long *__restrict__ bin_offsets, uint32_t *__restrict__ idx_out, uint32_t *__restrict__ part_tot,
@@ -596,7 +564,7 @@
     constexpr bool CAN_STAGE = STAGE && XM_SCATTER_STAGED != 0 && NSUB * 256 == XM_GRAN;
     __shared__ uint8_t lut_all[NIB ? 1 : XM_BLOCK / 64][64];
     __shared__ uint64_t lptr_all[LISTS ? XM_BLOCK / 64 : 1][8];
-    __shared__ __attribute__((aligned(16))) uint16_t slab_all[CAN_STAGE ? XM_BLOCK / 64 : 1][CAN_STAGE ? XM_SLAB_U16 : 4];
+    __shared__ __attribute__((aligned(16))) uint16_t slab_all[CAN_STAGE ? XM_BLOCK / 64 : 1][CAN_STAGE ? XM_SLAB_U16 + 8 : 8];
     const uint32_t lane = threadIdx.x & 63u;
     if (last) {
         const uint32_t n_parts = (n_gran + XM_PART_GRAN - 1u) / XM_PART_GRAN, cells = 8u * XM_PART_REPLICAS * n_parts;
@@ -614,13 +582,15 @@
     uint32_t lane_base, n_units;
     {
         const uint32_t tot = (lane < 8u) ? (uint32_t)bin_totals[lane] : 0u;
-        const uint32_t off = (lane < 7u) ? gran_off[(uint64_t)lane * gran_stride + g0] : 0u;
+        const uint32_t off = (lane < 7u) ? gran_off[(uint64_t)g0 * 8u + lane] : 0u;
         const uint32_t bin_start = wave_scan_incl(tot) - tot;
         lane_base = LISTS ? off : bin_start + off;
         n_units = LISTS ? lo.cap : lane_value(bin_start, 7);
         if (g0 == g_first && last && lane < 8u) bin_offsets[lane] = (LISTS && lane < 7u) ? tot : bin_start;
     }
     uint16_t *slab = slab_all[CAN_STAGE ? wave : 0];
+    const IndexSink to_out = {idx_out, n_units, slab, lptr};
+    const IndexSink to_slab = {idx_out, (uint32_t)XM_SLAB_U16, slab, lptr};
 
     auto load_granule = [&](uint32_t g, uint32_t w[NSUB]) {
         const uint64_t rec_g = (uint64_t)g * (NSUB * 256u);
@@ -659,30 +629,25 @@
         uint32_t run_start = 0, run_len = 0;
         bool staged = false;
         if (CAN_STAGE) {
-            const uint32_t cnt_g = (lane < 7u) ? gran_counts[(uint64_t)lane * gran_stride + g] : 0u;
+            const uint32_t cnt_g = (lane < 7u) ? gran_counts[(uint64_t)g * 8u + lane] : 0u;
             staged = slab_layout(cnt_g, run_start, run_len);
         }
-        uint32_t base[7];
-#pragma unroll
-        for (int b = 0; b < 7; ++b) base[b] = lane_value(staged ? run_start : lane_base, b);
+        uint32_t place = staged ? run_start : lane_base;
         const uint32_t rec_g = (uint32_t)((uint64_t)g * (NSUB * 256u));
         uint32_t w[NSUB];
         load_granule(g, w);
         if (!NIB || LISTS) lds_settle();
         if (CAN_STAGE && staged) {
-            scatter_granule<NSUB, WIDE, NIB, true, LISTS>(w, lut, rec_g, base, idx_out, n_units, slab, lptr);
+            scatter_granule<NSUB, WIDE, NIB, true, false>(w, lut, rec_g, place, to_slab);
             lds_settle();
             copy_runs_out(run_start, run_len, rec_g);
         } else {
-            scatter_granule<NSUB, WIDE, NIB, false, LISTS>(w, lut, rec_g, base, idx_out, n_units, slab, lptr);
+            scatter_granule<NSUB, WIDE, NIB, false, LISTS>(w, lut, rec_g, place, to_out);
         }
         return;
     }
 
     const uint32_t g1 = g0 + gran_per_wave < n_gran ? g0 + gran_per_wave : n_gran;
-    uint32_t base[7];
-#pragma unroll
-    for (int b = 0; b < 7; ++b) base[b] = lane_value(lane_base, b);
     uint32_t w[NSUB], wn[NSUB];
     load_granule(g0, w);
     if (!NIB || LISTS) lds_settle();
@@ -690,29 +655,20 @@
         if (g + 1u < g1) load_granule(g + 1u, wn);
         const uint32_t rec_g = (uint32_t)((uint64_t)g * (NSUB * 256u));
         bool staged = false;
-        uint32_t cnt_g = 0;
         if (CAN_STAGE) {
-            cnt_g = (lane < 7u) ? gran_counts[(uint64_t)lane * gran_stride + g] : 0u;
+            const uint32_t cnt_g = (lane < 7u) ? gran_counts[(uint64_t)g * 8u + lane] : 0u;
             uint32_t run_start, run_len;
             staged = slab_layout(cnt_g, run_start, run_len);
             if (staged) {
-                uint32_t sbase[7];
-#pragma unroll
-                for (int b = 0; b < 7; ++b) sbase[b] = lane_value(run_start, b);
-                scatter_granule<NSUB, WIDE, NIB, true, LISTS>(w, lut, rec_g, sbase, idx_out, n_units, slab, lptr);
+                uint32_t place = run_start;
+                scatter_granule<NSUB, WIDE, NIB, true, false>(w, lut, rec_g, place, to_slab);
                 lds_settle();
                 copy_runs_out(run_start, run_len, rec_g);
                 lds_settle();
+                lane_base += cnt_g;
             }
         }
-        if (!staged) {
-            if (CAN_STAGE) {
-#pragma unroll
-                for (int b = 0; b < 7; ++b) base[b] = lane_value(lane_base, b);
-            }
-            scatter_granule<NSUB, WIDE, NIB, false, LISTS>(w, lut, rec_g, base, idx_out, n_units, slab, lptr);
-        }
-        if (CAN_STAGE) lane_base += cnt_g;
+        if (!staged) scatter_granule<NSUB, WIDE, NIB, false, LISTS>(w, lut, rec_g, lane_base, to_out);
 #pragma unroll
         for (int s = 0; s < NSUB; ++s) w[s] = wn[s];
     }
@@ -773,6 +729,7 @@
     const uint32_t g = blockIdx.x;
     const uint64_t g4 = (uint64_t)blockIdx.x * BLOCK + threadIdx.x;
     const uint64_t r0 = g4 * 4;
+    const uint32_t first_bits = PAIRED ? reinterpret_cast<const uint32_t *>(unit_bits8)[(uint64_t)blockIdx.x * (BLOCK / 8)] : 0u;
     T a1[4], x1[4], a2[4], x2[4];
     load4<T, NT, FULL>(as1, r0, n, a1);
     load4<T, NT, FULL>(xs1, r0, n, x1);
@@ -782,13 +739,10 @@
     if (FULL || r0 < n) mb = (uint32_t)(unit_bits8[g4 >> 1] >> ((g4 & 1u) * 4u)) & 0xFu;
     if (!FULL && r0 + 4 > n) mb &= (r0 < n) ? ((1u << (uint32_t)(n - r0)) - 1u) : 0u;
     uint32_t halo = 0;
-    if (PAIRED && threadIdx.x == 0) {
-        if (r0 > 0) {
-            const uint64_t h = r0 - 1;
-            halo = mapping_state<T>(as1[h], xs1[h], as2[h], xs2[h], m);
-        } else {
-            mb &= ~1u;
-        }
+    if (PAIRED && r0 == 0) mb &= ~1u;
+    if (PAIRED && threadIdx.x == 0 && r0 > 0 && (!XM_HALO_WHEN_USED || (first_bits & 1u))) {
+        const uint64_t h = r0 - 1;
+        halo = mapping_state<T>(as1[h], xs1[h], as2[h], xs2[h], m);
     }
     uint32_t s[4];
 #pragma unroll
@@ -1156,7 +1110,7 @@
             mb &= ~1u;
         }
     }
-    const CountSink none = {nullptr, nullptr, nullptr, nullptr, 0u, 0, 0u};
+    const CountSink none = {nullptr, nullptr, nullptr, nullptr, 0, 0u};
     classify_finish<int32_t, PAIRED, BLOCK, FULL, false, -1>(a1, x1, a2, x2, m, mb, halo, last_state, code, r0, n, nullptr, none);
 }
 
@@ -1512,7 +1466,6 @@
     uint64_t g = (n + XM_GRAN - 1) / XM_GRAN;
     if (g == 0) g = 1;
     p.n_gran = (uint32_t)g;
-    p.gran_stride = (p.n_gran + 63u) & ~63u;
     return p;
 }
 
@@ -1523,7 +1476,6 @@
     s.part_tot = cp ? cp->part_tot : nullptr;
     s.counts_rep = cp ? reinterpret_cast<unsigned long long *>(cp->counts_rep) : nullptr;
     s.bins4 = cp ? cp->bins4 : nullptr;
-    s.gran_stride = cp ? cp->plan.gran_stride : 0u;
     s.mode = mode;
     s.blk0 = cp ? cp->gran0 : 0u;
     return s;
@@ -1655,8 +1607,8 @@
     unsigned long long *cnt = reinterpret_cast<unsigned long long *>(counts);
     const uint32_t part0 = cp.gran1 ? cp.gran0 / XM_PART_GRAN : 0u;
     const uint32_t part1 = cp.gran1 ? (cp.gran1 + XM_PART_GRAN - 1) / XM_PART_GRAN : n_parts;
-    scan_kernel<<<dim3(part1 - part0, 8), XM_SCAN_THREADS, 0, st>>>(cp.gran_counts, cp.gran1 ? cp.gran1 : cp.plan.n_gran, cp.plan.gran_stride,
-                                                                   cp.part_tot, gran_off, bt, rep, cnt, part0, n_parts);
+    scan_kernel<<<dim3(part1 - part0, 8), XM_SCAN_THREADS, 0, st>>>(cp.gran_counts, cp.gran1 ? cp.gran1 : cp.plan.n_gran,
+                                                           cp.part_tot, gran_off, bt, rep, cnt, part0, n_parts);
 }
 
 static uint32_t scatter_waves()
@@ -1682,7 +1634,7 @@
     const bool wide = n > (1ull << 30);
     const bool stage = mode == XM_MODE_SE;
     const ListOut lo = lists ? *lists : ListOut{{nullptr, nullptr, nullptr, nullptr, nullptr, nullptr, nullptr}, 0u};
-#define XM_LAUNCH_SCT(W, NIB, STG, L, M) scatter_kernel<XM_GRAN / 256, W, NIB, STG, L, M><<<grid, XM_BLOCK, 0, st>>>(code, n, mode, g_end, p.gran_stride, gran_counts, gran_off, bt, bo, idx_out, part_tot, lo, gran_per_wave, g_first, last)
+#define XM_LAUNCH_SCT(W, NIB, STG, L, M) scatter_kernel<XM_GRAN / 256, W, NIB, STG, L, M><<<grid, XM_BLOCK, 0, st>>>(code, n, mode, g_end, gran_counts, gran_off, bt, bo, idx_out, part_tot, lo, gran_per_wave, g_first, last)
 #define XM_LAUNCH_SCT0(W, NIB, STG, L) do { if (multi) XM_LAUNCH_SCT(W, NIB, STG, L, true); else XM_LAUNCH_SCT(W, NIB, STG, L, false); } while (0)
 #define XM_LAUNCH_SCT1(W, NIB, STG) do { if (lists) XM_LAUNCH_SCT0(W, NIB, STG, true); else XM_LAUNCH_SCT0(W, NIB, STG, false); } while (0)
 #define XM_LAUNCH_SCT2(W, NIB) do { if (stage) XM_LAUNCH_SCT1(W, NIB, true); else XM_LAUNCH_SCT1(W, NIB, false); } while (0)
diff --git a/xenomapper_amd/csrc/xm_ranks.h b/xenomapper_amd/csrc/xm_ranks.h
--- /dev/null
+++ b/xenomapper_amd/csrc/xm_ranks.h
@@ -0,0 +1,78 @@
+#pragma once
+#include <stdint.h>
+
+#if defined(__HIPCC__)
+#define XM_HD __host__ __device__ __forceinline__
+#else
+#define XM_HD inline
+#endif
+
+namespace xm {
+
+#define XM_RANK_BITS 9u
+#define XM_RANK_MASK 0x1FFu
+
+struct PackedUnits {
+    uint32_t lo, hi, b6;
+};
+
+XM_HD uint32_t rank_shift(uint32_t bin)
+{
+#if defined(__HIP_DEVICE_COMPILE__)
+    return __builtin_amdgcn_perm(0x3F3F3229u, 0x20120900u, bin);
+#else
+    return (uint32_t)(0x3F3F322920120900ull >> (8u * (bin & 7u))) & 0xFFu;
+#endif
+}
+
+XM_HD PackedUnits packed_add(PackedUnits a, PackedUnits b)
+{
+    PackedUnits r;
+    r.lo = a.lo + b.lo; r.hi = a.hi + b.hi; r.b6 = a.b6 + b.b6;
+    return r;
+}
+
+template <bool HAS6>
+XM_HD PackedUnits packed_one(uint32_t bin)
+{
+    const uint64_t one = 1ull << rank_shift(bin);
+    PackedUnits r;
+    r.lo = (uint32_t)one; r.hi = (uint32_t)(one >> 32);
+    r.b6 = (HAS6 && bin == 6u) ? 1u : 0u;
+    return r;
+}
+
+template <bool HAS6>
+XM_HD uint32_t packed_field(PackedUnits v, uint32_t bin)
+{
+    const uint64_t both = ((uint64_t)v.hi << 32) | v.lo;
+    const uint32_t f = (uint32_t)(both >> rank_shift(bin)) & XM_RANK_MASK;
+    return (HAS6 && bin == 6u) ? v.b6 : f;
+}
+
+template <bool HAS6>
+XM_HD uint32_t place_advance(PackedUnits totals, uint32_t lane)
+{
+    return lane < (HAS6 ? 7u : 6u) ? packed_field<HAS6>(totals, lane) : 0u;
+}
+
+template <int SLOTS, bool HAS6, typename Scan>
+XM_HD PackedUnits tile_ranks(const uint32_t bin[4], uint32_t rank[4], Scan scan)
+{
+    PackedUnits one[4], own = {0u, 0u, 0u};
+#pragma unroll
+    for (int j = 0; j < 4; ++j)
+        if ((SLOTS >> j) & 1) { one[j] = packed_one<HAS6>(bin[j]); own = packed_add(own, one[j]); }
+    PackedUnits incl;
+    incl.lo = scan(own.lo); incl.hi = scan(own.hi); incl.b6 = HAS6 ? scan(own.b6) : 0u;
+    PackedUnits run;
+    run.lo = incl.lo - own.lo; run.hi = incl.hi - own.hi; run.b6 = incl.b6 - own.b6;
+#pragma unroll
+    for (int j = 0; j < 4; ++j) {
+        rank[j] = 0u;
+        if ((SLOTS >> j) & 1) { rank[j] = packed_field<HAS6>(run, bin[j]); run = packed_add(run, one[j]); }
+    }
+    return incl;
+}
+
+}
```

Measured after the change: 149.6 billion read-pairs/s, median of 6. +4.0%, better.
